# sb17v/GaussianK-SGD

Hardware: AMD Instinct MI355X
Metric: images/sec (whole node) ResNet-50 k=0.1% at 1/2/4/8 MI355X; effective grad compression ratio (higher is better)
Workload: dtype fp32; 1 GPU; model=resnet50, global_batch=512, per_gpu_batch=512, image_size=224, parallelism=dp1, compressor=gaussian, buckets=1, threshold=524288000, planner=threshold, exchange=local, momentum_correction=True, hip_graph=False, f32_matmul=bf16x6

## Files before the change

gaussiank_sgd_amd/ops/bn.py:

```python
from __future__ import annotations

import os
from typing import Optional

import torch
import torch.nn as nn
import torch.nn.functional as F

from . import load, require_native

_CL = torch.channels_last
_FIN_FUSE = os.environ.get("GKSGD_BN_FIN_FUSE", "0") == "1"


def _ops():
    return torch.ops.gksgd


def _grad_pair(grads, like):
    gs = [g for g in grads if g is not None]
    out = []
    for g in gs:
        g = g.contiguous(memory_format=_CL)
        if g.dtype != like.dtype:
            g = g.to(like.dtype)
        out.append(g)
    return (out + [None, None])[:2]


class BnLink:

    __slots__ = ("h", "mask", "twin", "dy2", "dz", "part", "dy2c", "geo")

    def __init__(self):
        self.h = self.mask = self.dy2 = self.dz = self.part = self.dy2c = self.geo = None
        self.twin = False

    def ready(self) -> bool:
        return self.h is not None and (not self.twin or self.dy2 is not None)

    def scatter_dy2c(self) -> Optional[torch.Tensor]:
        if self.dy2c is None:
            return None
        H, W, OH, OW = self.geo
        C = self.dy2c.shape[1]
        N = self.dy2c.shape[0] // (OH * OW)
        full = torch.empty((N, C, H, W), dtype=self.dy2c.dtype, device=self.dy2c.device, memory_format=_CL).zero_()
        full[:, :, ::2, ::2] = self.dy2c.view(N, OH, OW, C).permute(0, 3, 1, 2)
        return full

    def clear(self) -> None:
        self.h = self.mask = self.dy2 = self.dz = self.part = self.dy2c = self.geo = None


class ProducerLink:

    __slots__ = ("lazy", "dx")

    def __init__(self):
        self.lazy = None
        self.dx = None

    def matches(self, dy: torch.Tensor) -> bool:
        return self.lazy is not None and dy.data_ptr() == self.lazy[0].data_ptr() and dy.shape == self.lazy[0].shape

    def materialize(self) -> torch.Tensor:
        if self.dx is None:
            dz, x, coef, _, _ = self.lazy
            self.dx = torch.empty_like(x, memory_format=_CL)
            _ops().bn_lazy_apply(dz, x, self.dx, coef)
        return self.dx

    def clear(self) -> None:
        self.lazy = self.dx = None


def _lazy_buffers(x: torch.Tensor):
    C = x.shape[1]
    coef = torch.empty(C, 4, dtype=torch.float32, device=x.device)
    padz = torch.empty(C, dtype=x.dtype, device=x.device)
    padx = torch.empty(C, dtype=x.dtype, device=x.device)
    return coef, padz, padx


def _lazy_ok(x: torch.Tensor, plink) -> bool:
    import os
    return (plink is not None and x.dtype == torch.float32 and x.shape[1] % 64 == 0 and
            os.environ.get("GKSGD_BN_LAZY", "0") != "0")


class _BNActFn(torch.autograd.Function):
    @staticmethod
    def forward(ctx, x, residual, weight, bias, running_mean, running_var, momentum, eps, relu, direct=None,
                nbt=None, twin=False, pre=None, link=None, res_link=None, plink=None, fin=None, rbn=None):
        ctx.direct = direct
        ctx.set_materialize_grads(False)
        C = x.shape[1]
        M = x.numel() // C
        eb = x.element_size()
        y = torch.empty_like(x, memory_format=_CL)
        stats = torch.empty(4, C, dtype=torch.float32, device=x.device)
        ws = torch.empty(int(_ops().bn_workspace_floats(M, C, eb)), dtype=torch.float32, device=x.device)
        rscale, rshift, dlink = rbn if rbn is not None else (None, None, None)
        ctx.dlink = dlink
        if rbn is not None and (residual.dtype != x.dtype or not residual.is_contiguous(memory_format=_CL)):
            raise RuntimeError("deferred residual BN: the pending tensor must match x (dtype, channels-last)")
        if residual is not None and residual.dtype != x.dtype:
            residual = residual.to(x.dtype)
        if residual is not None and not residual.is_contiguous(memory_format=_CL):
            residual = residual.contiguous(memory_format=_CL)
        mask = None
        if relu:
            mask = torch.empty(int(_ops().bn_mask_bytes(M, C, eb)), dtype=torch.uint8, device=x.device)
        pre_t, pre_rows = pre if pre is not None else (None, 0)
        _ops().bn_act_forward(x, residual, y, mask, weight, bias, running_mean, running_var, stats[0], stats[1],
                              stats[2], stats[3], ws, float(eps), float(momentum), bool(relu), nbt, pre_t, pre_rows,
                              fin, rscale, rshift)
        ctx.fin = fin
        ctx.relu = bool(relu)
        ctx.has_res = residual is not None
        ctx.save_for_backward(x, mask, weight, stats[0], stats[1])
        ctx.link = link
        ctx.res_link = res_link
        ctx.plink = plink
        if link is not None:
            link.h, link.mask, link.twin = x, mask, bool(twin)
        return (y, y.view_as(y)) if twin else y

    @staticmethod
    def backward(ctx, *grads):
        x, mask, weight, mean, invstd = ctx.saved_tensors
        link, res_link, plink, dlink = ctx.link, ctx.res_link, ctx.plink, ctx.dlink
        ctx.link = ctx.res_link = ctx.plink = ctx.dlink = None
        gw, gb = ctx.direct if ctx.direct is not None else (None, None)
        lazy = _lazy_ok(x, plink) and ctx.needs_input_grad[0]
        if link is not None and link.part is not None:
            dz = grads[0]
            if dz is None or dz.data_ptr() != link.dz.data_ptr():
                raise RuntimeError("BNAct bwd_link: the linked output had another consumer")
            part, rows = link.part
            link.clear()
            g = torch.empty(2, x.shape[1], dtype=torch.float32, device=x.device)
            if lazy:
                coef, padz, padx = _lazy_buffers(x)
                _ops().bn_bwd_lazy_pre(x, part, rows, weight, mean, invstd, g[0], g[1], coef, padz, padx, gw, gb)
                plink.lazy = (dz, x, coef, padz, padx)
                dx = dz
            elif dlink is not None and ctx.needs_input_grad[1]:
                dx = torch.empty_like(x, memory_format=_CL)
                x2 = dlink.x
                dx2 = torch.empty_like(x2, memory_format=_CL)
                g2 = torch.empty(2, x2.shape[1], dtype=torch.float32, device=x.device)
                ws2 = torch.empty(int(_ops().bn_workspace_floats(x2.numel() // x2.shape[1], x2.shape[1],
                                                                 x2.element_size())),
                                  dtype=torch.float32, device=x.device)
                gw2, gb2 = dlink.direct if dlink.direct is not None else (None, None)
                _ops().bn_act_backward_pre_dual(dz, x, dx, weight, mean, invstd, g[0], g[1], part, rows, gw, gb, x2,
                                                dx2, dlink.weight, dlink.mean, dlink.invstd, g2[0], g2[1], ws2, gw2,
                                                gb2)
                dlink.dz, dlink.dx, dlink.g = dz, dx2, g2
            else:
                dx = torch.empty_like(x, memory_format=_CL)
                _ops().bn_act_backward_pre(dz, x, dx, weight, mean, invstd, g[0], g[1], part, rows, gw, gb, ctx.fin)
            dres = dz if ctx.has_res and ctx.needs_input_grad[1] else None
            if res_link is not None and dres is not None:
                res_link.dy2 = dres
            if ctx.direct is not None:
                return (dx, dres) + (None,) * 16
            dgamma = g[0] if weight is not None and ctx.needs_input_grad[2] else None
            dbeta = g[1] if ctx.needs_input_grad[3] else None
            return (dx, dres, dgamma, dbeta) + (None,) * 14
        d2c = link.scatter_dy2c() if link is not None else None
        if link is not None:
            link.clear()
        dy, dy2 = _grad_pair(tuple(grads) + (d2c,), x)
        if dy is None:
            return (None,) * 18
        C = x.shape[1]
        M = x.numel() // C
        g = torch.empty(2, C, dtype=torch.float32, device=x.device)
        ws = torch.empty(int(_ops().bn_workspace_floats(M, C, x.element_size())), dtype=torch.float32,
                         device=x.device)
        if lazy:
            dz = torch.empty_like(x, memory_format=_CL)
            coef, padz, padx = _lazy_buffers(x)
            _ops().bn_act_backward_lazy(dy, dy2, mask, x, dz, weight, mean, invstd, g[0], g[1], ws, ctx.relu, coef,
                                        padz, padx, gw, gb)
            plink.lazy = (dz, x, coef, padz, padx)
            dx = dz
            dres = dz if ctx.has_res and ctx.needs_input_grad[1] else None
        else:
            dx = torch.empty_like(x, memory_format=_CL)
            dres = torch.empty_like(x, memory_format=_CL) if ctx.has_res and ctx.needs_input_grad[1] else None
            _ops().bn_act_backward(dy, mask, x, dx, dres, weight, mean, invstd, g[0], g[1], ws, ctx.relu, gw, gb,
                                   dy2, ctx.fin)
        if res_link is not None and dres is not None:
            res_link.dy2 = dres
        if ctx.direct is not None:
            return (dx, dres) + (None,) * 16
        dgamma = g[0] if weight is not None and ctx.needs_input_grad[2] else None
        dbeta = g[1] if ctx.needs_input_grad[3] else None
        return (dx, dres, dgamma, dbeta) + (None,) * 14


class DeferLink:

    __slots__ = ("x", "weight", "mean", "invstd", "direct", "dz", "dx", "g")

    def __init__(self, x, weight, mean, invstd, direct):
        self.x, self.weight, self.mean, self.invstd, self.direct = x, weight, mean, invstd, direct
        self.dz = self.dx = self.g = None


class _BNDeferFn(torch.autograd.Function):

    @staticmethod
    def forward(ctx, x, weight, bias, running_mean, running_var, momentum, eps, stats, direct=None, nbt=None,
                pre=None, dlink=None):
        ctx.direct = direct
        ctx.set_materialize_grads(False)
        C = x.shape[1]
        M = x.numel() // C
        ws = torch.empty(int(_ops().bn_workspace_floats(M, C, x.element_size())), dtype=torch.float32,
                         device=x.device)
        pre_t, pre_rows = pre if pre is not None else (None, 0)
        _ops().bn_act_finalize(x, weight, bias, running_mean, running_var, stats[0], stats[1], stats[2], stats[3], ws,
                               float(eps), float(momentum), nbt, pre_t, pre_rows)
        ctx.save_for_backward(x, weight, stats[0], stats[1])
        ctx.dlink = dlink
        return x.view_as(x)

    @staticmethod
    def backward(ctx, dy):
        x, weight, mean, invstd = ctx.saved_tensors
        dl, ctx.dlink = ctx.dlink, None
        if dy is None:
            return (None,) * 12
        if dl is not None and dl.dx is not None and dl.dz is not None and dy.data_ptr() == dl.dz.data_ptr():
            dx, g = dl.dx, dl.g
            dl.dz = dl.dx = dl.g = None
            if ctx.direct is not None:
                return (dx,) + (None,) * 11
# ... 210 lines not shown
```

gaussiank_sgd_amd/ops/conv1x1.py:

```python
from __future__ import annotations

import os
from itertools import product
from typing import Dict

import torch
import torch.nn as nn
import torch.nn.functional as F

from . import autotune
from . import load
from . import streams
from . import weight_prep
from .autotune import (X6, f32_matmul, load_choices, save_choices, set_f32_matmul,
                       tuned_choices, tuning_log)

_CL = torch.channels_last
_ENABLED = os.environ.get("GKSGD_FASTCONV", "1") != "0"
_BIAS_COLSUM = os.environ.get("GKSGD_CONV_BIAS_COLSUM", "1") != "0"
_WINO = os.environ.get("GKSGD_WINO", "1") != "0"
_FORCE = os.environ.get("GKSGD_CONV_FORCE", "")
_WINO_GRIDS = (0, 1 << 20)
_zeros: Dict[torch.device, torch.Tensor] = {}

# ... 129 lines not shown
def _lz_kw(lz, rows: bool = False) -> dict:
    _, x, coef, padz, padx = lz
    return dict(lz_x=_rows(x) if rows else x, lz_coef=coef, lz_padz=padz, lz_padx=padx)


def _dgrad(dy: torch.Tensor, w: torch.Tensor, x_shape, s: int, lz=None, plink=None, wp: bool = False) -> torch.Tensor:
    N, C, H, W, K, k, p, OH, OW = _geom(x_shape, w, s)
    g = _g()
    dt = dy.dtype
    xs = torch.empty(x_shape, dtype=dt, device=dy.device, memory_format=_CL)
    kw = _lz_kw(lz, rows=(s == 1 and k == 1)) if lz is not None else {}

    def miopen():
        return torch.ops.aten.convolution_backward(dy, xs, w, None, [s, s], [p, p], [1, 1], False, [0, 0], 1,
                                                   [True, False, False])[0]
    cands = []
    split = []
    dx = None
    if s == 2:
        dx = xs
        z = _zero(dy.device)
        run = lambda c, mb: g.conv_dgrad_s2(dy, w, dx, z, c, mb, **kw)
        cands = autotune.hip_cands(run, product(autotune.nt_cfgs(dt), autotune.NT_GRIDS))
    if s == 1:
        dx = xs
        if k == 1:
            DY, DX = _rows(dy), _rows(dx)
            Wt = _lazy(lambda: weight_prep.transposed_1x1(w, wp))
            run = lambda c, mb: g.gemm_nt(DY, Wt(), DX, c, mb, **kw)
            if lz is None:
                split = autotune.splitk_cfgs(dt, N * H * W, C, K)
        else:
            wf = _lazy(lambda: weight_prep.flipped_3x3(w, wp))
            z = _zero(dy.device)
            run = lambda c, mb: g.conv_nt(dy, wf(), dx, z, 1, p, c, mb, **kw)
        cands = autotune.hip_cands(run, product(autotune.nt_cfgs(dt), autotune.NT_GRIDS))
        cands += autotune.hip_cands(run, product(split, autotune.SPLITK_GRIDS))
    if lz is not None:
        cands.append((("mat", 0, 0), lambda: _dgrad(plink.materialize(), w, x_shape, s, wp=wp)))
        ch = autotune.pick(("dgrad", N, C, H, W, K, k, s) + autotune.dkey(dt) + ("lz",), cands)
        if ch[0] == "mat":
            return _dgrad(plink.materialize(), w, x_shape, s, wp=wp)
        run(ch[1], ch[2])
        return dx
    wino = _wino_ok(dt, k, s, K, C) and _wino_shape_fits(N, H, W, C, K)
    if wino:
        cands += _wino_cands(dy, w, dx, True, wp=wp)
    cands.append((("miopen", 0, 0), miopen))
    ch = autotune.pick(_dgrad_key(N, C, H, W, K, k, s, dt), _forced(cands))
    if ch[0] == "miopen":
        return miopen().contiguous(memory_format=_CL)
    if ch[0] in ("wino", "wx6"):
        dict(cands)[ch]()
        return dx
    run(ch[1], ch[2])
    return dx


_WGRAD_AFTER = os.environ.get("GKSGD_WGRAD_AFTER_DGRAD", "0") == "1"
_SIDE_QROUNDS = int(os.environ.get("GKSGD_WGRAD_SIDE_QROUNDS", "0"))
_FORK_BIAS = os.environ.get("GKSGD_WGRAD_STREAM_BIAS", "0") == "1"
_FORKABLE = tuple(k for k in os.environ.get("GKSGD_WGRAD_STREAM_KINDS", "hip,w3,wino").split(",")
                  if k and (k != "wino" or os.environ.get("GKSGD_WGRAD_STREAM_WINO", "1") == "1"))


def _lazy(make):
    box = []

    def get():
        if not box:
            box.append(make())
        return box[0]
    return get


def _dgrad_key(N, C, H, W, K, k, s, dt) -> tuple:
    wino = _wino_ok(dt, k, s, K, C) and _wino_shape_fits(N, H, W, C, K)
    return ("dgrad", N, C, H, W, K, k, s) + autotune.dkey(dt) + (_wino_tag(K, C) if wino else ())


def _dgrad_bn(dy: torch.Tensor, w: torch.Tensor, x_shape, s: int, link, lz=None, plink=None,
              wp: bool = False) -> torch.Tensor:
    N, C, H, W, K, k, p, OH, OW = _geom(x_shape, w, s)
    kw = _lz_kw(lz, rows=(k == 1)) if lz is not None else {}
    g = _g()
    M = N * H * W
    dt = dy.dtype
    dz = torch.empty(x_shape, dtype=dt, device=dy.device, memory_format=_CL)
    st = torch.empty(2, min(1280, (M + 63) // 64), C, dtype=torch.float32, device=dy.device)
    h, mask, dy2 = link.h, link.mask, link.dy2
    if k == 1:
        DY, DZ = _rows(dy), _rows(dz)
        Wt = _lazy(lambda: weight_prep.transposed_1x1(w, wp))
        H2 = _rows(h)
        D2 = _rows(dy2) if dy2 is not None else None
        run = lambda c, mb: g.gemm_nt(DY, Wt(), DZ, c, mb, st, None, H2, D2, mask, **kw)
        split = autotune.splitk_cfgs(dt, M, C, K) if lz is None else []
    else:
        split = []
        wf = _lazy(lambda: weight_prep.flipped_3x3(w, wp))
        z = _zero(dy.device)
        run = lambda c, mb: g.conv_nt(dy, wf(), dz, z, 1, p, c, mb, st, None, h, dy2, mask, **kw)
    bn_cfgs = [c for c in autotune.nt_cfgs(dt) if c % 10 <= 4 or c >= 1000]
    cands = autotune.hip_cands(run, product(bn_cfgs, autotune.NT_GRIDS))
    cands += autotune.hip_cands(run, product(split, autotune.SPLITK_GRIDS))
    key = ("dgrad_bn", N, C, H, W, K, k, s, dy2 is not None) + autotune.dkey(dt)
    if lz is not None:
        cands.append((("mat", 0, 0), lambda: _dgrad_bn(plink.materialize(), w, x_shape, s, link, wp=wp)))
        ch = autotune.pick(key + ("lz",), cands)
        if ch[0] == "mat":
            return _dgrad_bn(plink.materialize(), w, x_shape, s, link, wp=wp)
    else:
        if _wino_ok(dt, k, s, K, C) and _wino_shape_fits(N, H, W, C, K):
            cands += _wino_cands(dy, w, dz, True, st, (h, dy2, mask), wp=wp)
            key = key + _wino_tag(K, C)
        ch = autotune.pick(key, _forced(cands))
    if ch[0] in ("wino", "wx6"):
        rows = dict(cands)[ch]()
    else:
        rows = run(ch[1], ch[2])
    link.part = (st, int(rows))
    link.dz = dz
    return dz


def _link_on(ds: bool = False) -> bool:
    return os.environ.get("GKSGD_BN_LINK", "1") != "0" and \
        not (ds and os.environ.get("GKSGD_BN_LINK_DS", "1") == "0")


def _ds_compact_ok(ds_link, x: torch.Tensor, w: torch.Tensor, s: int, dt: torch.dtype) -> bool:
    return (ds_link is not None and s == 2 and w.shape[2] == 1 and dt == torch.float32 and _link_on(ds=True) and
            f32_matmul() == "bf16x6" and ds_link.h is not None and ds_link.h.dtype == dt and
            ds_link.h.shape == x.shape and ds_link.dy2 is None and ds_link.dy2c is None and
            x.numel() // x.shape[1] < (1 << 31))


def _dgrad_ds(dy: torch.Tensor, w: torch.Tensor, x_shape, wp: bool = False) -> torch.Tensor:
    N, C, H, W, K, k, p, OH, OW = _geom(x_shape, w, 2)
    g = _g()
    dt = dy.dtype
    dxc = torch.empty(N * OH * OW, C, dtype=dt, device=dy.device)
    DY = _rows(dy)
    Wt = _lazy(lambda: weight_prep.transposed_1x1(w, wp))
    run = lambda c, mb: g.gemm_nt(DY, Wt(), dxc, c, mb)
    cands = autotune.hip_cands(run, product(autotune.nt_cfgs(dt), autotune.NT_GRIDS))
    cands += autotune.hip_cands(run, product(autotune.splitk_cfgs(dt, N * OH * OW, C, K), autotune.SPLITK_GRIDS))
    ch = autotune.pick(("dgrad_ds", N, C, H, W, K) + autotune.dkey(dt), cands)
    run(ch[1], ch[2])
    return dxc


def _ds_fusable(link, x: torch.Tensor, w: torch.Tensor, s: int, dt: torch.dtype, dgrad_key: tuple, lz) -> bool:
    if not (s == 1 and w.shape[2] == 1 and dt == torch.float32 and lz is None and _link_on(ds=True) and
            f32_matmul() == "bf16x6" and link.h is not None and link.h.dtype == dt and link.h.shape == x.shape):
        return False
    ch = autotune.choice(dgrad_key)
    return ch is None or ch[0] == "hip"


def _dgrad_bn_ds(dy: torch.Tensor, w: torch.Tensor, x_shape, link, wp: bool = False) -> torch.Tensor:
    N, C, H, W, K, k, p, OH, OW = _geom(x_shape, w, 1)
    g = _g()
    M = N * H * W
    dt = dy.dtype
    dz = torch.empty(x_shape, dtype=dt, device=dy.device, memory_format=_CL)
    st = torch.empty(2, min(1280, (M + 63) // 64), C, dtype=torch.float32, device=dy.device)
    DY, DZ, H2 = _rows(dy), _rows(dz), _rows(link.h)
    D2, geo, mask = link.dy2c, list(link.geo), link.mask
    Wt = _lazy(lambda: weight_prep.transposed_1x1(w, wp))
    run = lambda c, mb: g.gemm_nt(DY, Wt(), DZ, c, mb, st, None, H2, D2, mask, bn_dy2_geo=geo)
    cands = autotune.hip_cands(run, product(autotune.nt_x62_cfgs(), autotune.NT_GRIDS))
    ch = autotune.pick(("dgrad_bn_ds", N, C, H, W, K) + autotune.dkey(dt), cands)
    rows = run(ch[1], ch[2])
    link.part = (st, int(rows))
    link.dz = dz
    link.dy2c = None
    return dz


def _bn_fusable(link, s: int, dgrad_key: tuple) -> bool:
    if link is None or s != 1 or not _link_on() or not link.ready():
        return False
    if link.h.dtype != dgrad_key_dtype(dgrad_key):
        return False
    ch = autotune.choice(dgrad_key)
    return ch is None or ch[0] in ("hip", "wino", "wx6")


def dgrad_key_dtype(key: tuple) -> torch.dtype:
    return torch.float32 if "f32" in key[8:] else torch.bfloat16


def _wgrad_key(x: torch.Tensor, w: torch.Tensor, s: int, lz=None) -> tuple:
    N, C, H, W, K, k, p, OH, OW = _geom(x.shape, w, s)
    wino = lz is None and _wino_ok(x.dtype, k, s, C, K) and C % 64 == 0 and _wino_shape_fits(N, H, W, C, K)
    return ("wgrad", N, C, H, W, K, k, s) + autotune.dkey(x.dtype) + (("lz",) if lz is not None else ()) + \
        (("wino",) if wino else ())


def _wgrad_into(dy: torch.Tensor, x: torch.Tensor, w: torch.Tensor, s: int, out_f32: torch.Tensor, lz=None,
                plink=None, side: bool = False) -> None:
    N, C, H, W, K, k, p, OH, OW = _geom(x.shape, w, s)
    g = _g()
# ... 247 lines not shown
```

gaussiank_sgd_amd/ops/csrc/bindings.cpp:

```cpp
#include <ATen/ATen.h>
#include <c10/core/DeviceGuard.h>
#include <c10/hip/HIPStream.h>
#include <torch/custom_class.h>
#include <torch/library.h>

#include <cstring>
#include <vector>

#include "comm/rccl_engine.h"
#include "kernels/gemm_cfg.h"
#include "kernels/gk_kernels.h"

namespace {

hipStream_t cur_stream(const at::Tensor& t) {
  return c10::hip::getCurrentHIPStream(t.device().index()).stream();
}

void check_dev(const at::Tensor& t, const char* name) {
  TORCH_CHECK(t.is_cuda(), name, " must be a GPU tensor");
  TORCH_CHECK(t.is_contiguous(), name, " must be contiguous");
}

void check_f32(const at::Tensor& t, const char* name) {
// ... 511 lines not shown
  return (int64_t)gk::bn_mask_bytes(M, (int)C, (int)elem_bytes);
}

void* fin_state(const OptTensor& fin, int C) {
  if (!has(fin)) return nullptr;
  TORCH_CHECK(fin->is_cuda() && fin->is_contiguous() && fin->nbytes() >= gk::bn_fin_state_bytes(C) &&
                  reinterpret_cast<uintptr_t>(fin->data_ptr()) % 16 == 0,
              "fin: a contiguous, 16-byte aligned GPU tensor of bn_fin_state_bytes(C) bytes");
  return fin->data_ptr();
}

int64_t bn_fin_state_bytes(int64_t C) { return (int64_t)gk::bn_fin_state_bytes((int)C); }

void bn_act_forward(at::Tensor x, OptTensor res, at::Tensor y, OptTensor mask, OptTensor w, OptTensor b,
                    OptTensor run_mean, OptTensor run_var, at::Tensor save_mean, at::Tensor save_invstd,
                    at::Tensor scale, at::Tensor shift, at::Tensor ws, double eps, double momentum, bool relu,
                    OptTensor nbt, OptTensor pre, int64_t pre_rows, OptTensor fin, OptTensor rscale,
                    OptTensor rshift) {
  const gk::BnShape sh = bn_shape(x);
  check_same(x, {&y}, "y");
  gk::BnResidual r{opt_same(x, res, "residual"), nullptr, nullptr};
  TORCH_CHECK(has(rscale) == has(rshift), "rscale and rshift go together");
  if (has(rscale)) {
    TORCH_CHECK(r.res != nullptr, "rscale / rshift need a residual");
    r.rscale = opt_channel_buf(rscale, sh.C, "rscale");
    r.rshift = opt_channel_buf(rshift, sh.C, "rshift");
  }
  const gk::BnFwdStats st =
      fwd_stats(w, b, run_mean, run_var, save_mean, save_invstd, scale, shift, eps, momentum, nbt, sh.C);
  float* wp = check_ws(ws, sh);
  uint8_t* mp = relu_mask(mask, relu, sh);
  const gk::BnPartials p = partials(pre, pre_rows, sh.C, "pre");
  void* fs = fin_state(fin, sh.C);
  c10::DeviceGuard guard(x.device());
  gk::bn_act_forward(sh, x.data_ptr(), r, y.data_ptr(), mp, st, p, wp, relu ? 1 : 0, fs, cur_stream(x));
}

void bn_act_finalize(at::Tensor x, OptTensor w, OptTensor b, OptTensor run_mean, OptTensor run_var,
                     at::Tensor save_mean, at::Tensor save_invstd, at::Tensor scale, at::Tensor shift, at::Tensor ws,
                     double eps, double momentum, OptTensor nbt, OptTensor pre, int64_t pre_rows) {
  const gk::BnShape sh = bn_shape(x);
  const gk::BnFwdStats st =
      fwd_stats(w, b, run_mean, run_var, save_mean, save_invstd, scale, shift, eps, momentum, nbt, sh.C);
  float* wp = check_ws(ws, sh);
  const gk::BnPartials p = partials(pre, pre_rows, sh.C, "pre");
  c10::DeviceGuard guard(x.device());
  gk::bn_act_finalize(sh, x.data_ptr(), st, p, wp, cur_stream(x));
}

void bn_act_backward(at::Tensor dy, OptTensor mask, at::Tensor x, at::Tensor dx, OptTensor dres, OptTensor w,
                     at::Tensor mean, at::Tensor invstd, at::Tensor dgamma, at::Tensor dbeta, at::Tensor ws, bool relu,
                     OptTensor gw_acc, OptTensor gb_acc, OptTensor dy2, OptTensor fin) {
  const gk::BnShape sh = bn_shape(x);
  check_same(x, {&dy}, "dy");
  check_same(x, {&dx}, "dx");
  void* rp = opt_same(x, dres, "dres");
  const void* d2 = opt_dy2(dy2, dy);
  const gk::BnBwdStats bs = bwd_stats(w, mean, invstd, dgamma, dbeta, gw_acc, gb_acc, sh.C);
  float* wp = check_ws(ws, sh);
  const uint8_t* mp = relu_mask(mask, relu, sh);
  void* fs = fin_state(fin, sh.C);
  c10::DeviceGuard guard(x.device());
  gk::bn_act_backward(sh, dy.data_ptr(), d2, mp, x.data_ptr(), dx.data_ptr(), rp, bs, wp, relu ? 1 : 0, fs,
                      cur_stream(x));
}

void bn_act_backward_pre(at::Tensor dz, at::Tensor x, at::Tensor dx, OptTensor w, at::Tensor mean, at::Tensor invstd,
                         at::Tensor dgamma, at::Tensor dbeta, at::Tensor part, int64_t rows, OptTensor gw_acc,
                         OptTensor gb_acc, OptTensor fin) {
  const gk::BnShape sh = bn_shape(x);
  check_same(x, {&dz}, "dz");
  check_same(x, {&dx}, "dx");
  const gk::BnBwdStats bs = bwd_stats(w, mean, invstd, dgamma, dbeta, gw_acc, gb_acc, sh.C);
  const gk::BnPartials p = partials(part, rows, sh.C, "part");
  void* fs = fin_state(fin, sh.C);
  c10::DeviceGuard guard(x.device());
  gk::bn_act_backward_pre(sh, dz.data_ptr(), x.data_ptr(), dx.data_ptr(), bs, p, fs, cur_stream(x));
}

void bn_act_backward_pre_dual(at::Tensor dz, at::Tensor x, at::Tensor dx, OptTensor w, at::Tensor mean,
                              at::Tensor invstd, at::Tensor dgamma, at::Tensor dbeta, at::Tensor part, int64_t rows,
                              OptTensor gw_acc, OptTensor gb_acc, at::Tensor x2, at::Tensor dx2, OptTensor w2,
                              at::Tensor mean2, at::Tensor invstd2, at::Tensor dgamma2, at::Tensor dbeta2,
                              at::Tensor ws2, OptTensor gw2_acc, OptTensor gb2_acc) {
  const gk::BnShape sh = bn_shape(x);
  check_same(x, {&dz, &dx, &x2, &dx2}, "dz / dx / x2 / dx2");
  const gk::BnBwdStats bs = bwd_stats(w, mean, invstd, dgamma, dbeta, gw_acc, gb_acc, sh.C);
  const gk::BnBwdStats bs2 = bwd_stats(w2, mean2, invstd2, dgamma2, dbeta2, gw2_acc, gb2_acc, sh.C);
  const gk::BnPartials p = partials(part, rows, sh.C, "part");
  float* wp2 = check_ws(ws2, sh);
  c10::DeviceGuard guard(x.device());
  gk::bn_act_backward_pre_dual(sh, dz.data_ptr(), x.data_ptr(), dx.data_ptr(), bs, p, x2.data_ptr(), dx2.data_ptr(),
                               bs2, wp2, cur_stream(x));
}

gk::BnLazyOut lazy_out(const at::Tensor& x, int C, const at::Tensor& coef, const at::Tensor& padz,
                       const at::Tensor& padx) {
  TORCH_CHECK(coef.is_cuda() && coef.scalar_type() == at::kFloat && coef.is_contiguous() && coef.numel() >= 4 * C,
              "coef must be a contiguous fp32 [C, 4] GPU tensor");
  for (const at::Tensor* t : {&padz, &padx})
    TORCH_CHECK(t->is_cuda() && t->scalar_type() == x.scalar_type() && t->is_contiguous() && t->numel() >= C,
                "padz / padx must be contiguous [C] GPU tensors of x's dtype");
  return {coef.data_ptr<float>(), padz.data_ptr(), padx.data_ptr()};
}

void bn_bwd_lazy_pre(at::Tensor x, at::Tensor part, int64_t rows, OptTensor w, at::Tensor mean, at::Tensor invstd,
                     at::Tensor dgamma, at::Tensor dbeta, at::Tensor coef, at::Tensor padz, at::Tensor padx,
                     OptTensor gw_acc, OptTensor gb_acc) {
  const gk::BnShape sh = bn_shape(x);
  const gk::BnPartials p = partials(part, rows, sh.C, "part");
  const gk::BnBwdStats bs = bwd_stats(w, mean, invstd, dgamma, dbeta, gw_acc, gb_acc, sh.C);
  const gk::BnLazyOut lz = lazy_out(x, sh.C, coef, padz, padx);
  c10::DeviceGuard guard(x.device());
  gk::bn_bwd_finalize_lazy(sh, p, 1, bs, lz, cur_stream(x));
}

void bn_act_backward_lazy(at::Tensor dy, OptTensor dy2, OptTensor mask, at::Tensor x, at::Tensor dz, OptTensor w,
                          at::Tensor mean, at::Tensor invstd, at::Tensor dgamma, at::Tensor dbeta, at::Tensor ws,
                          bool relu, at::Tensor coef, at::Tensor padz, at::Tensor padx, OptTensor gw_acc,
                          OptTensor gb_acc) {
  const gk::BnShape sh = bn_shape(x);
  check_same(x, {&dy}, "dy");
  check_same(x, {&dz}, "dz");
  const void* d2 = opt_dy2(dy2, dy);
  const gk::BnBwdStats bs = bwd_stats(w, mean, invstd, dgamma, dbeta, gw_acc, gb_acc, sh.C);
  float* wp = check_ws(ws, sh);
  const uint8_t* mp = relu_mask(mask, relu, sh);
  const gk::BnLazyOut lz = lazy_out(x, sh.C, coef, padz, padx);
  c10::DeviceGuard guard(x.device());
  gk::bn_act_backward_lazy(sh, dy.data_ptr(), d2, mp, x.data_ptr(), dz.data_ptr(), bs, wp, relu ? 1 : 0, lz,
                           cur_stream(x));
}

void bn_stats_partials(at::Tensor x, at::Tensor ws) {
  const gk::BnShape sh = bn_shape(x);
  float* wp = check_ws(ws, sh);
  c10::DeviceGuard guard(x.device());
  gk::bn_stats_partials(sh, x.data_ptr(), wp, cur_stream(x));
}

void bn_lazy_apply(at::Tensor dz, at::Tensor x, at::Tensor dx, at::Tensor coef) {
  const gk::BnShape sh = bn_shape(x);
  check_same(x, {&dz}, "dz");
  check_same(x, {&dx}, "dx");
  TORCH_CHECK(coef.is_cuda() && coef.scalar_type() == at::kFloat && coef.is_contiguous() && coef.numel() >= 4 * sh.C,
              "coef must be a contiguous fp32 [C, 4] GPU tensor");
  c10::DeviceGuard guard(x.device());
  gk::bn_lazy_apply(sh, dz.data_ptr(), x.data_ptr(), dx.data_ptr(), coef.data_ptr<float>(), cur_stream(x));
}

gk::PoolGeo pool_geo(const at::Tensor& x, const at::Tensor& y, const char* y_name, int64_t k, int64_t st,
                     int64_t pad) {
  check_cl(y, y_name);
  TORCH_CHECK(x.dim() == 4 && y.dim() == 4 && x.size(0) == y.size(0) && x.size(1) == y.size(1) &&
                  y.scalar_type() == x.scalar_type(),
              y_name, " must be 4-D with x's batch, channels and dtype");
  gk::PoolGeo pg;
  pg.H = (int)x.size(2);
  pg.W = (int)x.size(3);
  pg.OH = (int)y.size(2);
  pg.OW = (int)y.size(3);
  pg.k = (int)k;
  pg.s = (int)st;
  pg.p = (int)pad;
  TORCH_CHECK(k >= 1 && k <= 15 && st >= 1 && pad >= 0 && 2 * pad <= k, "unsupported pool window");
  TORCH_CHECK(pg.OH == (pg.H + 2 * pg.p - pg.k) / pg.s + 1 && pg.OW == (pg.W + 2 * pg.p - pg.k) / pg.s + 1,
              "pool output shape mismatch (ceil_mode unsupported)");
  TORCH_CHECK(x.numel() / x.size(1) < (int64_t(1) << 32), "N*H*W must be < 2^32");
  return pg;
}

uint8_t* pool_amax(const at::Tensor& amax, const at::Tensor& y) {
  TORCH_CHECK(amax.is_cuda() && amax.scalar_type() == at::kByte && amax.numel() >= y.numel(),
              "amax: a uint8 GPU tensor of the pooled tensor's element count");
  return amax.data_ptr<uint8_t>();
}
// ... 111 lines not shown
  void init_async(at::Tensor uid, int64_t rank, int64_t world, int64_t device) {
    TORCH_CHECK(!uid.is_cuda() && uid.scalar_type() == at::kByte, "uid must be a CPU uint8 tensor");
    at::Tensor c = uid.contiguous();
    std::vector<uint8_t> v(c.data_ptr<uint8_t>(), c.data_ptr<uint8_t>() + c.numel());
    comm.init_async(v, (int)rank, (int)world, (int)device);
  }
  int64_t init_poll() { return comm.init_poll(); }
  void init_wait(double timeout_s) { comm.init_wait(timeout_s); }
  void abort() { comm.abort(); }
  void set_op_timeout(double s) { comm.set_op_timeout(s); }

  void allgather(at::Tensor send, at::Tensor recv) {
    check_dev(send, "send");
    check_dev(recv, "recv");
    TORCH_CHECK(recv.nbytes() == send.nbytes() * (size_t)comm.world(), "recv must be world x send bytes");
    c10::DeviceGuard guard(send.device());
    comm.allgather_bytes(send.data_ptr(), recv.data_ptr(), send.nbytes(), cur_stream(send));
  }

  void allreduce(at::Tensor t, int64_t op) {
    check_dev(t, "t");
    c10::DeviceGuard guard(t.device());
    ncclRedOp_t o = op == 0 ? ncclSum : (op == 1 ? ncclAvg : (op == 2 ? ncclMax : ncclMin));
    comm.allreduce(t.data_ptr(), (size_t)t.numel(), to_nccl(t.scalar_type()), o, cur_stream(t));
  }

  void broadcast(at::Tensor t, int64_t root) {
    check_dev(t, "t");
    c10::DeviceGuard guard(t.device());
    comm.broadcast(t.data_ptr(), (size_t)t.numel(), to_nccl(t.scalar_type()), (int)root, cur_stream(t));
  }

  void allgather_many(std::vector<at::Tensor> sends, std::vector<at::Tensor> recvs) {
    TORCH_CHECK(sends.size() == recvs.size() && !sends.empty(), "allgather_many: matching non-empty lists");
    std::vector<const void*> sp;
    std::vector<void*> rp;
    std::vector<size_t> nb;
    for (size_t i = 0; i < sends.size(); ++i) {
      check_dev(sends[i], "send");
      check_dev(recvs[i], "recv");
      TORCH_CHECK(sends[i].device() == sends[0].device() && recvs[i].device() == sends[0].device(),
                  "allgather_many: one device");
      TORCH_CHECK(recvs[i].nbytes() == sends[i].nbytes() * (size_t)comm.world(), "recv must be world x send bytes");
      sp.push_back(sends[i].data_ptr());
      rp.push_back(recvs[i].data_ptr());
      nb.push_back(sends[i].nbytes());
    }
    c10::DeviceGuard guard(sends[0].device());
    comm.allgather_many(sp, rp, nb, cur_stream(sends[0]));
  }

  void inject_failure(std::string why) { comm.inject_failure(why); }
  void destroy() { comm.destroy(); }
  int64_t rank() const { return comm.rank(); }
  int64_t world() const { return comm.world(); }

  void set_tracking(bool on) { comm.set_tracking(on); }
  void start_watchdog(double timeout_s, double poll_ms) { comm.start_watchdog(timeout_s, poll_ms); }
  void stop_watchdog() { comm.stop_watchdog(); }
  int64_t poll() { return comm.poll(); }
  bool failed() const { return comm.failed(); }
  std::string error() const { return comm.error(); }
  void check() const { comm.check(); }
  int64_t in_flight() const { return comm.in_flight(); }
  void reset_stats() { comm.reset_stats(); }
  std::vector<double> stats(int64_t op) const {
    gk::OpStats st = comm.stats((int)op);
    return {(double)st.calls, (double)st.bytes, st.ms_total, st.ms_max};
  }
};

bool gemm_supported(int64_t N, int64_t K) { return gk::gemm_supported(N, K); }

bool is_gemm_dtype(const at::Tensor& t) { return t.scalar_type() == at::kBFloat16 || t.scalar_type() == at::kFloat; }

void check_rows(const at::Tensor& t, const char* name, const at::Tensor& like) {
  TORCH_CHECK(t.is_cuda() && is_gemm_dtype(t) && t.scalar_type() == like.scalar_type() && t.dim() == 2, name,
              " must be a 2-D bf16 or fp32 GPU tensor (all operands one dtype)");
  TORCH_CHECK(t.stride(1) == 1 && (t.stride(0) * t.element_size()) % 16 == 0, name,
              " rows must be contiguous, 16-byte aligned");
  TORCH_CHECK(reinterpret_cast<uintptr_t>(t.data_ptr()) % 16 == 0, name, " must be 16-byte aligned");
}

float* stats_ptr(const c10::optional<at::Tensor>& st, int64_t N, int* rows) {
  if (!st.has_value()) {
    *rows = 0;
    return nullptr;
  }
  const at::Tensor& t = *st;
  TORCH_CHECK(t.is_cuda() && t.scalar_type() == at::kFloat && t.is_contiguous() && t.dim() == 3 && t.size(0) == 2 &&
                  t.size(2) == N && t.size(1) > 0,
              "stats must be a contiguous fp32 [2, rows, N] GPU tensor");
  *rows = (int)t.size(1);
  return t.data_ptr<float>();
}

void check_stem_x(const at::Tensor& x) {
  TORCH_CHECK(x.is_cuda() && x.dim() == 4 && x.size(1) == 3 &&
                  (x.scalar_type() == at::kFloat || x.scalar_type() == at::kBFloat16) &&
                  x.is_contiguous(at::MemoryFormat::ChannelsLast),
              "stem: x must be a channels-last fp32 / bf16 [N, 3, H, W] GPU tensor");
  TORCH_CHECK(gk::stem_supported((int)x.size(2), (int)x.size(3)), "stem: unsupported image size");
  TORCH_CHECK(x.size(0) * x.size(2) * x.size(3) < (int64_t(1) << 31), "stem: batch too large");
}

void stem_pack(at::Tensor w, at::Tensor wp) {
  TORCH_CHECK(w.is_cuda() && w.scalar_type() == at::kFloat && w.dim() == 4 && w.size(0) == 64 && w.size(1) == 3 &&
                  w.size(2) == 7 && w.size(3) == 7,
              "stem_pack: w must be fp32 [64, 3, 7, 7]");
  TORCH_CHECK(wp.is_cuda() && wp.scalar_type() == at::kBFloat16 && wp.is_contiguous() && wp.numel() == 64 * 224,
              "stem_pack: wp must be contiguous bf16 [64, 224]");
  c10::DeviceGuard guard(w.device());
  gk::stem_pack_weight(w.data_ptr<float>(), w.stride(0), w.stride(1), w.stride(2), w.stride(3),
                       static_cast<uint16_t*>(wp.data_ptr()), cur_stream(w));
}

int64_t stem_fwd(at::Tensor x, at::Tensor wp, at::Tensor y, c10::optional<at::Tensor> stats) {
  check_stem_x(x);
  const int64_t N = x.size(0), H = x.size(2), W = x.size(3);
  const int64_t OH = (H - 1) / 2 + 1, OW = (W - 1) / 2 + 1;
  TORCH_CHECK(wp.is_cuda() && wp.scalar_type() == at::kBFloat16 && wp.is_contiguous() && wp.numel() == 64 * 224,
              "stem_fwd: wp must be the packed bf16 [64, 224] weights");
  TORCH_CHECK(y.is_cuda() && y.scalar_type() == at::kBFloat16 && y.dim() == 4 && y.size(0) == N && y.size(1) == 64 &&
                  y.size(2) == OH && y.size(3) == OW && y.is_contiguous(at::MemoryFormat::ChannelsLast),
              "stem_fwd: y must be channels-last bf16 [N, 64, OH, OW]");
  int rows = 0;
  float* sp = stats_ptr(stats, 64, &rows);
  c10::DeviceGuard guard(x.device());
  return gk::stem_forward(x.data_ptr(), x.scalar_type() == at::kFloat, (int)N, (int)H, (int)W,
                          static_cast<const uint16_t*>(wp.data_ptr()), static_cast<uint16_t*>(y.data_ptr()), sp, rows,
                          cur_stream(x));
}

int64_t stem_wgrad_ws(int64_t N, int64_t H, int64_t W) {
  return (int64_t)gk::stem_wgrad_blocks((int)N, (int)H, (int)W) * 64 * 224;
}

void stem_wgrad(at::Tensor x, at::Tensor dy, at::Tensor out, at::Tensor part) {
  check_stem_x(x);
  const int64_t N = x.size(0), H = x.size(2), W = x.size(3);
  const int64_t OH = (H - 1) / 2 + 1, OW = (W - 1) / 2 + 1;
  TORCH_CHECK(dy.is_cuda() && dy.scalar_type() == at::kBFloat16 && dy.dim() == 4 && dy.size(0) == N &&
                  dy.size(1) == 64 && dy.size(2) == OH && dy.size(3) == OW &&
                  dy.is_contiguous(at::MemoryFormat::ChannelsLast),
              "stem_wgrad: dy must be channels-last bf16 [N, 64, OH, OW]");
  TORCH_CHECK(out.is_cuda() && out.scalar_type() == at::kFloat && out.dim() == 4 && out.size(0) == 64 &&
                  out.size(1) == 3 && out.size(2) == 7 && out.size(3) == 7,
              "stem_wgrad: out must be fp32 [64, 3, 7, 7]");
  TORCH_CHECK(part.is_cuda() && part.scalar_type() == at::kFloat && part.is_contiguous() &&
                  part.numel() >= stem_wgrad_ws(N, H, W),
              "stem_wgrad: part must hold stem_wgrad_ws(N, H, W) floats");
  c10::DeviceGuard guard(x.device());
  gk::stem_wgrad(x.data_ptr(), x.scalar_type() == at::kFloat, (int)N, (int)H, (int)W,
                 static_cast<const uint16_t*>(dy.data_ptr()), part.data_ptr<float>(), out.data_ptr<float>(),
                 out.stride(0), out.stride(1), out.stride(2), out.stride(3), cur_stream(x));
}

int64_t stem_f32_fwd(at::Tensor x, at::Tensor w, at::Tensor y, c10::optional<at::Tensor> stats) {
  TORCH_CHECK(x.is_cuda() && x.scalar_type() == at::kFloat && x.dim() == 4 && x.size(1) == 3 &&
                  x.is_contiguous(at::MemoryFormat::ChannelsLast) && gk::stem_f32_supported((int)x.size(2), (int)x.size(3)) &&
                  reinterpret_cast<uintptr_t>(x.data_ptr()) % 16 == 0,
              "stem_f32_fwd: x must be a channels-last fp32 [N, 3, 224, 224] GPU tensor (16-byte aligned)");
  TORCH_CHECK(w.is_cuda() && w.scalar_type() == at::kFloat && w.dim() == 4 && w.size(0) == 64 && w.size(1) == 3 &&
                  w.size(2) == 7 && w.size(3) == 7, "stem_f32_fwd: w must be fp32 [64, 3, 7, 7]");
  const int64_t N = x.size(0);
  TORCH_CHECK(y.is_cuda() && y.scalar_type() == at::kFloat && y.dim() == 4 && y.size(0) == N && y.size(1) == 64 &&
                  y.size(2) == 112 && y.size(3) == 112 && y.is_contiguous(at::MemoryFormat::ChannelsLast),
              "stem_f32_fwd: y must be a channels-last fp32 [N, 64, 112, 112] GPU tensor");
  int rows = 0;
  float* sp = stats_ptr(stats, 64, &rows);
  c10::DeviceGuard guard(x.device());
  return gk::stem_f32_forward(x.data_ptr<float>(), (int)N, (int)x.size(2), (int)x.size(3), w.data_ptr<float>(),
                              w.stride(0), w.stride(1), w.stride(2), w.stride(3), y.data_ptr<float>(), sp, rows,
                              cur_stream(x));
}

int64_t stem_f32x6_wplanes() { return gk::stem_f32x6_wplanes(); }

int64_t stem_f32x6_fwd(at::Tensor x, at::Tensor w, at::Tensor y, c10::optional<at::Tensor> stats, at::Tensor wp3) {
  TORCH_CHECK(x.is_cuda() && x.scalar_type() == at::kFloat && x.dim() == 4 && x.size(1) == 3 &&
                  x.is_contiguous(at::MemoryFormat::ChannelsLast) && gk::stem_f32_supported((int)x.size(2), (int)x.size(3)) &&
                  reinterpret_cast<uintptr_t>(x.data_ptr()) % 16 == 0,
              "stem_f32x6_fwd: x must be a channels-last fp32 [N, 3, 224, 224] GPU tensor (16-byte aligned)");
  TORCH_CHECK(w.is_cuda() && w.scalar_type() == at::kFloat && w.dim() == 4 && w.size(0) == 64 && w.size(1) == 3 &&
                  w.size(2) == 7 && w.size(3) == 7, "stem_f32x6_fwd: w must be fp32 [64, 3, 7, 7]");
  const int64_t N = x.size(0);
  TORCH_CHECK(y.is_cuda() && y.scalar_type() == at::kFloat && y.dim() == 4 && y.size(0) == N && y.size(1) == 64 &&
                  y.size(2) == 112 && y.size(3) == 112 && y.is_contiguous(at::MemoryFormat::ChannelsLast),
              "stem_f32x6_fwd: y must be a channels-last fp32 [N, 64, 112, 112] GPU tensor");
  TORCH_CHECK(wp3.is_cuda() && wp3.scalar_type() == at::kBFloat16 && wp3.is_contiguous() &&
                  wp3.numel() >= gk::stem_f32x6_wplanes() && reinterpret_cast<uintptr_t>(wp3.data_ptr()) % 16 == 0,
              "stem_f32x6_fwd: wp3 must be a contiguous bf16 GPU tensor of stem_f32x6_wplanes() elements");
  int rows = 0;
  float* sp = stats_ptr(stats, 64, &rows);
  c10::DeviceGuard guard(x.device());
  return gk::stem_f32x6_forward(x.data_ptr<float>(), (int)N, (int)x.size(2), (int)x.size(3), w.data_ptr<float>(),
                                w.stride(0), w.stride(1), w.stride(2), w.stride(3),
                                static_cast<uint16_t*>(wp3.data_ptr()), y.data_ptr<float>(), sp, rows, cur_stream(x));
}

int64_t stem_f32_wgrad_ws(int64_t N) { return (int64_t)gk::stem_f32_wgrad_blocks((int)N) * 64 * 148; }

void stem_f32_wgrad(at::Tensor x, at::Tensor dy, at::Tensor out, at::Tensor part, bool x6) {
  TORCH_CHECK(x.is_cuda() && x.scalar_type() == at::kFloat && x.dim() == 4 && x.size(1) == 3 &&
                  x.is_contiguous(at::MemoryFormat::ChannelsLast) && gk::stem_f32_supported((int)x.size(2), (int)x.size(3)) &&
                  reinterpret_cast<uintptr_t>(x.data_ptr()) % 16 == 0,
              "stem_f32_wgrad: x must be a channels-last fp32 [N, 3, 224, 224] GPU tensor (16-byte aligned)");
  const int64_t N = x.size(0);
  TORCH_CHECK(dy.is_cuda() && dy.scalar_type() == at::kFloat && dy.dim() == 4 && dy.size(0) == N &&
                  dy.size(1) == 64 && dy.size(2) == 112 && dy.size(3) == 112 &&
                  dy.is_contiguous(at::MemoryFormat::ChannelsLast),
              "stem_f32_wgrad: dy must be a channels-last fp32 [N, 64, 112, 112] GPU tensor");
  TORCH_CHECK(out.is_cuda() && out.scalar_type() == at::kFloat && out.dim() == 4 && out.size(0) == 64 &&
                  out.size(1) == 3 && out.size(2) == 7 && out.size(3) == 7, "stem_f32_wgrad: out must be fp32 [64, 3, 7, 7]");
  TORCH_CHECK(part.is_cuda() && part.scalar_type() == at::kFloat && part.is_contiguous() &&
                  part.numel() >= stem_f32_wgrad_ws(N), "stem_f32_wgrad: part must hold stem_f32_wgrad_ws(N) floats");
  c10::DeviceGuard guard(x.device());
  gk::stem_f32_wgrad(x.data_ptr<float>(), dy.data_ptr<float>(), (int)N, (int)x.size(2), (int)x.size(3),
                     part.data_ptr<float>(), out.data_ptr<float>(), out.stride(0), out.stride(1), out.stride(2),
                     out.stride(3), x6, cur_stream(x));
}

const uint32_t* seed_word(const c10::optional<at::Tensor>& t) {
  if (!t.has_value() || !t->defined()) return nullptr;
  TORCH_CHECK(t->is_cuda() && t->scalar_type() == at::kInt && t->numel() >= 1, "seed_dev must be a GPU int32[>=1]");
  return reinterpret_cast<const uint32_t*>(t->data_ptr<int32_t>());
}

const float* bias_ptr(const c10::optional<at::Tensor>& b, int64_t N) {
  if (!b.has_value() || !b->defined()) return nullptr;
  TORCH_CHECK(b->is_cuda() && b->scalar_type() == at::kFloat && b->is_contiguous() && b->numel() == N,
              "bias must be a contiguous fp32 [N] GPU tensor");
  return b->data_ptr<float>();
}

bool bn_bwd_args(const c10::optional<at::Tensor>& h, const c10::optional<at::Tensor>& dy2,
                 const c10::optional<at::Tensor>& mask, int64_t M, int64_t N,
                 int64_t ldc, bool has_stats, at::ScalarType dt, gk::BnBwdArgs* out,
                 c10::OptionalArrayRef<int64_t> dy2_geo = c10::nullopt) {
  const bool compact = dy2_geo.has_value();
  if (!h.has_value() || !h->defined()) {
    TORCH_CHECK(!compact, "bn_dy2_geo needs the BN-backward epilogue operands");
    return false;
  }
  TORCH_CHECK(has_stats, "BN-backward epilogue needs the stats partials buffer");
  auto rows_ok = [&](const at::Tensor& t, const char* what) {
    TORCH_CHECK(t.is_cuda() && t.scalar_type() == dt && t.numel() == M * N &&
                    (t.dim() == 2 ? t.stride(0) == ldc && t.stride(1) == 1
                                  : t.is_contiguous(at::MemoryFormat::ChannelsLast) && ldc == N),
                what, " must have C's dtype, shape and row stride");
  };
  rows_ok(*h, "bn h");
  out->h = h->data_ptr();
  out->dy2 = nullptr;
  out->H = out->W = out->OH = out->OW = 0;
  if (compact) {
    TORCH_CHECK(dy2_geo->size() == 4 && dy2.has_value() && dy2->defined(), "bn_dy2_geo is [H, W, OH, OW] of a given bn_dy2");
    const int64_t H = (*dy2_geo)[0], W = (*dy2_geo)[1], OH = (*dy2_geo)[2], OW = (*dy2_geo)[3];
    TORCH_CHECK(H > 0 && W > 0 && OH == (H + 1) / 2 && OW == (W + 1) / 2 && M % (H * W) == 0 && M < (int64_t(1) << 31),
                "bn_dy2_geo: OH x OW must be the stride-2 grid of the H x W pixels of C's rows (M < 2^31)");
    TORCH_CHECK(dt == at::kFloat && dy2->is_cuda() && dy2->scalar_type() == dt && dy2->dim() == 2 &&
                    dy2->size(0) == M / (H * W) * OH * OW && dy2->size(1) == N && dy2->stride(0) == ldc &&
                    dy2->stride(1) == 1,
                "compact bn dy2 must be fp32 [M / (H W) * OH * OW, N] with C's row stride");
    out->dy2 = dy2->data_ptr();
    out->H = (int)H, out->W = (int)W, out->OH = (int)OH, out->OW = (int)OW;
  } else if (dy2.has_value() && dy2->defined()) {
    rows_ok(*dy2, "bn dy2");
    out->dy2 = dy2->data_ptr();
  }
  out->mask = nullptr;
  if (mask.has_value() && mask->defined()) {
    const int64_t V = dt == at::kFloat ? 4 : 8;
    TORCH_CHECK(mask->is_cuda() && mask->scalar_type() == at::kByte && mask->numel() >= M * (N / V),
                "bn mask must hold M * N / V bytes");
    out->mask = mask->data_ptr<uint8_t>();
  }
  return true;
}

bool lazy_args(const c10::optional<at::Tensor>& x, const c10::optional<at::Tensor>& coef,
               const c10::optional<at::Tensor>& padz, const c10::optional<at::Tensor>& padx, const at::Tensor& dz,
               int64_t C, gk::LazyArgs* out) {
  if (!x.has_value() || !x->defined()) return false;
  TORCH_CHECK(dz.scalar_type() == at::kFloat, "lazy BN operand: fp32 kernels only");
  TORCH_CHECK(x->is_cuda() && x->scalar_type() == dz.scalar_type() && x->sizes() == dz.sizes() &&
                  x->strides() == dz.strides(),
              "lz_x must match the dz operand's dtype, shape and strides");
  TORCH_CHECK(coef.has_value() && coef->defined() && coef->is_cuda() && coef->scalar_type() == at::kFloat &&
                  coef->is_contiguous() && coef->numel() >= 4 * C,
              "lz_coef must be a contiguous fp32 [C, 4] GPU tensor");
  for (const c10::optional<at::Tensor>* t : {&padz, &padx})
    TORCH_CHECK(t->has_value() && (*t)->defined() && (*t)->is_cuda() && (*t)->scalar_type() == dz.scalar_type() &&
                    (*t)->is_contiguous() && (*t)->numel() >= C,
                "lz_padz / lz_padx must be contiguous [C] GPU tensors of dz's dtype");
  TORCH_CHECK(C > 0 && C % 64 == 0, "lazy BN operand: channels must be a multiple of 64");
  out->x = x->data_ptr();
  out->coef = coef->data_ptr<float>();
  out->padz = padz->data_ptr();
  out->padx = padx->data_ptr();
  out->C = (int)C;
  return true;
}

struct NtWordAux {
  at::Tensor ws, b3;
  NtWordAux(const char* op, const gk::cfg::NtWord& w, bool gather, bool f32, bool has_lz, const at::Tensor& B,
            int64_t ldb, int64_t M, int64_t N, int64_t K, int64_t C, hipStream_t stream) {
    if (w.planes > 1) {
      TORCH_CHECK(f32 && !has_lz && w.planes <= 16 && gk::cfg::splitk_divides(w.planes, gather, (int)K, (int)C), op,
                  " split-K: fp32, no lazy operand, S <= 16 ", gather ? "dividing the K slices" : "and K % (64 S) == 0");
      ws = at::empty({w.planes, M, N}, B.options().dtype(at::kFloat));
    }
    if (w.family == 3) {
      TORCH_CHECK(B.scalar_type() == at::kFloat && (gather || K % 32 == 0), op, ": cfg family 3 takes fp32 operands");
      b3 = at::empty({N, 3 * K}, B.options().dtype(at::kBFloat16));
      gk::split3_rows(B.data_ptr<float>(), ldb, b3.data_ptr(), N, (int)K, stream);
    }
  }
  float* ws_ptr() const { return ws.defined() ? ws.data_ptr<float>() : nullptr; }
  const void* b3_ptr() const { return b3.defined() ? b3.data_ptr() : nullptr; }
  static int64_t checked(const char* op, int r) {
    TORCH_CHECK(r != gk::cfg::kRowGemmsOnly, op,
                ": the register-staged bf16x6 kernels (cfg digit 200000/300000) take plain row GEMMs only");
    TORCH_CHECK(r != gk::cfg::kCompactDy2, op,
                ": a compact bn_dy2 takes one register-staged bf16x6 row GEMM (cfg digit 200000/300000, no split-K)");
    TORCH_CHECK(r >= 0, op, ": the lazy operand's coefficient table does not fit this tile configuration");
    return r;
  }
};

int64_t gemm_nt(at::Tensor A, at::Tensor B, at::Tensor C, int64_t cfg, int64_t max_blocks,
                c10::optional<at::Tensor> stats, c10::optional<at::Tensor> bias, c10::optional<at::Tensor> bn_h,
                c10::optional<at::Tensor> bn_dy2, c10::optional<at::Tensor> bn_mask, c10::optional<at::Tensor> lz_x, c10::optional<at::Tensor> lz_coef,
                c10::optional<at::Tensor> lz_padz, c10::optional<at::Tensor> lz_padx,
                c10::OptionalArrayRef<int64_t> bn_dy2_geo) {
  check_rows(A, "A", A);
  check_rows(B, "B", A);
  check_rows(C, "C", A);
  const int64_t M = A.size(0), K = A.size(1), N = B.size(0);
  TORCH_CHECK(B.size(1) == K && C.size(0) == M && C.size(1) == N, "gemm_nt: shape mismatch");
  TORCH_CHECK(gk::gemm_supported(N, K), "gemm_nt: N and K must be multiples of 64");
  TORCH_CHECK(M > 0, "gemm_nt: empty M");
  int rows = 0;
  float* sp = stats_ptr(stats, N, &rows);
  gk::BnBwdArgs bn{};
  const bool has_bn = bn_bwd_args(bn_h, bn_dy2, bn_mask, M, N, C.stride(0), sp != nullptr, C.scalar_type(), &bn,
                                  bn_dy2_geo);
  TORCH_CHECK(!has_bn || !bias.has_value() || !bias->defined(), "gemm_nt: bias and BN epilogue are exclusive");
  gk::LazyArgs lz{};
  const bool has_lz = lazy_args(lz_x, lz_coef, lz_padz, lz_padx, A, K, &lz);
  c10::DeviceGuard guard(A.device());
  const bool f32 = A.scalar_type() == at::kFloat;
  const NtWordAux aux("gemm_nt", gk::cfg::NtWord::decode((int)cfg), false, f32, has_lz, B, B.stride(0), M, N, K, K,
                      cur_stream(A));
  const int r = gk::gemm_nt(A.data_ptr(), A.stride(0), B.data_ptr(), B.stride(0), C.data_ptr(), C.stride(0), M, (int)N,
                            (int)K, f32, (int)cfg, (int)max_blocks, sp, rows, bias_ptr(bias, N),
                            has_bn ? &bn : nullptr, has_lz ? &lz : nullptr, cur_stream(A), aux.ws_ptr(), aux.b3_ptr());
  return NtWordAux::checked("gemm_nt", r);
}

void gemm_tn_acc(at::Tensor G, at::Tensor X, at::Tensor W, int64_t cfg, int64_t splits, c10::optional<at::Tensor> lz_x, c10::optional<at::Tensor> lz_coef,
                c10::optional<at::Tensor> lz_padz, c10::optional<at::Tensor> lz_padx) {
  check_rows(G, "G", G);
  check_rows(X, "X", G);
  TORCH_CHECK(W.is_cuda() && W.scalar_type() == at::kFloat && W.dim() == 2 && W.stride(1) == 1,
              "W must be a 2-D fp32 GPU tensor with contiguous rows");
  const int64_t M = G.size(0), N = G.size(1), K = X.size(1);
  TORCH_CHECK(X.size(0) == M && W.size(0) == N && W.size(1) == K, "gemm_tn_acc: shape mismatch");
  TORCH_CHECK(gk::gemm_supported(N, K), "gemm_tn_acc: N and K must be multiples of 64");
  if (M == 0) return;
  gk::LazyArgs lz{};
  const bool has_lz = lazy_args(lz_x, lz_coef, lz_padz, lz_padx, G, N, &lz);
  c10::DeviceGuard guard(G.device());
  const int rc = gk::gemm_tn_acc(G.data_ptr(), G.stride(0), X.data_ptr(), X.stride(0), W.data_ptr<float>(), W.stride(0), M, (int)N,
                  (int)K, G.scalar_type() == at::kFloat, (int)cfg, (int)splits, has_lz ? &lz : nullptr, cur_stream(G));
  TORCH_CHECK(rc != gk::cfg::kRowGemmsOnly, "gemm_tn_acc: the register-staged bf16x6 kernels (cfg digit 200000) take plain row GEMMs only");
}

void check_zero(const at::Tensor& zero) {
  TORCH_CHECK(zero.is_cuda() && zero.is_contiguous() && zero.numel() * zero.element_size() >= 128,
              "zero must hold >= 128 zero bytes");
}

void check_conv(const at::Tensor& x, const at::Tensor& w, const at::Tensor& zero) {
  TORCH_CHECK(x.is_cuda() && is_gemm_dtype(x) && x.dim() == 4 && x.is_contiguous(at::MemoryFormat::ChannelsLast),
              "conv: x must be a channels-last bf16 or fp32 GPU tensor");
  TORCH_CHECK(w.is_cuda() && w.scalar_type() == x.scalar_type() && w.dim() == 4 &&
                  w.is_contiguous(at::MemoryFormat::ChannelsLast) && w.size(1) == x.size(1),
              "conv: w must be a channels-last [Cout, C, KH, KW] GPU tensor of x's dtype");
  TORCH_CHECK(x.size(1) % 64 == 0 && w.size(0) % 64 == 0, "conv: C and Cout must be multiples of 64");
  check_zero(zero);
}

int64_t conv_nt(at::Tensor x, at::Tensor w, at::Tensor y, at::Tensor zero, int64_t stride, int64_t pad, int64_t cfg,
                int64_t max_blocks, c10::optional<at::Tensor> stats, c10::optional<at::Tensor> bias,
                c10::optional<at::Tensor> bn_h, c10::optional<at::Tensor> bn_dy2, c10::optional<at::Tensor> bn_mask,
                c10::optional<at::Tensor> lz_x, c10::optional<at::Tensor> lz_coef,
                c10::optional<at::Tensor> lz_padz, c10::optional<at::Tensor> lz_padx) {
  check_conv(x, w, zero);
  const int64_t N = x.size(0), C = x.size(1), H = x.size(2), W = x.size(3);
  const int64_t Co = w.size(0), KH = w.size(2), KW = w.size(3);
  const int64_t OH = (H + 2 * pad - KH) / stride + 1, OW = (W + 2 * pad - KW) / stride + 1;
  TORCH_CHECK(KH <= 4 && KW <= 4, "conv_nt: kernels up to 4x4 (gemm.hip kMaxTaps)");
  TORCH_CHECK(y.is_cuda() && y.scalar_type() == x.scalar_type() && y.dim() == 4 &&
                  y.is_contiguous(at::MemoryFormat::ChannelsLast) && y.size(0) == N && y.size(1) == Co &&
                  y.size(2) == OH && y.size(3) == OW,
              "conv_nt: y must be channels-last [N, Cout, OH, OW] of x's dtype");
  const int64_t M = N * OH * OW;
  TORCH_CHECK(M > 0 && M < (int64_t(1) << 32), "conv_nt: M out of range");
  int rows = 0;
  float* sp = stats_ptr(stats, Co, &rows);
  gk::BnBwdArgs bn{};
  const bool has_bn = bn_bwd_args(bn_h, bn_dy2, bn_mask, M, Co, Co, sp != nullptr, y.scalar_type(), &bn);
  TORCH_CHECK(!has_bn || !bias.has_value() || !bias->defined(), "conv_nt: bias and BN epilogue are exclusive");
  gk::LazyArgs lz{};
  const bool has_lz = lazy_args(lz_x, lz_coef, lz_padz, lz_padx, x, C, &lz);
  c10::DeviceGuard guard(x.device());
  const bool f32 = x.scalar_type() == at::kFloat;
  const int64_t K = KH * KW * C;
  const NtWordAux aux("conv_nt", gk::cfg::NtWord::decode((int)cfg), true, f32, has_lz, w, K, M, Co, K, C, cur_stream(x));
  const int r = gk::conv_nt(x.data_ptr(), zero.data_ptr(), (int)H, (int)W, (int)C, (int)OH, (int)OW, (int)stride,
                            (int)pad, (int)KH, (int)KW, w.data_ptr(), y.data_ptr(), M, (int)Co, f32, (int)cfg,
                            (int)max_blocks, sp, rows, bias_ptr(bias, Co), has_bn ? &bn : nullptr,
                            has_lz ? &lz : nullptr, cur_stream(x), aux.ws_ptr(), aux.b3_ptr());
  return NtWordAux::checked("conv_nt", r);
}

int64_t weight_prep_blocks(int64_t kind, int64_t R, int64_t S) { return gk::weight_prep_blocks((int)kind, (int)R, (int)S); }

void weight_prep(at::Tensor table, int64_t ndesc, int64_t total_blocks) {
// ... 668 lines not shown
    gk::lstm_cell_bwd(static_cast<const uint16_t*>(po), static_cast<const uint16_t*>(pr), pp, (int)S, pc,
                      gates.data_ptr<float>(), c.data_ptr<float>(), c_prev.data_ptr<float>(),
                      static_cast<uint16_t*>(dG.data_ptr()), static_cast<uint16_t*>(gp), dc_prev.data_ptr<float>(),
                      (int)B, (int)H, (int)Hp, cur_stream(gates));
}

}


TORCH_LIBRARY(gksgd, m) {
  m.def("ctrl_bytes() -> int", &ctrl_bytes);
  m.def("workspace_bytes() -> int", &workspace_bytes);
  m.def(
      "compress(Tensor(a!) g, Tensor(b!) r, Tensor(c!) ctrl, Tensor(d!) ws, Tensor(e!) record, int mode, bool ec, "
      "bool zero_g, int loops, float z, float fixed_thr, float sample_p, int k, int k_cap, int seed, "
      "int n_stats, Tensor(f!)? stats_out=None, Tensor? valid=None, Tensor(g!)? u=None, Tensor? w=None, "
      "Tensor? chunks=None, int chunk_begin=0, int chunk_count=0, int chunk_base=0, float[] mc_mu=[], "
      "float[] mc_wd=[], Tensor? seed_dev=None, int handoff=-1) -> ()");
  m.def("apply_records_sgd(Tensor(a!) w, Tensor(b!)? w_bf16, Tensor records, int P, int k_cap, float scale, float lr, "
        "Tensor? lr_mult=None) -> ()");
  m.def("arena_digest(Tensor x, Tensor(a!) out, Tensor(b!) ws) -> ()");
  m.def("tensor_stats(Tensor x, Tensor(a!) ctrl, Tensor(b!) ws) -> ()");
  m.def("quality_workspace_bytes() -> int", &quality_workspace_bytes);
  m.def("selection_quality(Tensor r, Tensor record, int k, int k_cap, Tensor(a!) out, Tensor(b!) ws) -> ()");
  m.def("scatter_add_records(Tensor(a!) dst, Tensor records, int P, int k_cap, float scale, bool deterministic) -> ()");
  m.def("fill_zero(Tensor(a!) dst) -> ()");
  m.def("sign_bucket_workspace_bytes() -> int", &sign_bucket_workspace_bytes);
  m.def("sign_bucket_compress(Tensor(a!) x, Tensor(b!) mask, Tensor(c!) means, Tensor(d!) ws) -> ()");
  m.def("sign_bucket_decompress(Tensor(a!) x, Tensor mask, Tensor means) -> ()");
  m.def(
      "fused_sgd(Tensor(a!) w, Tensor(b!)? m, Tensor(c!) g, Tensor chunks, float[] lr, float[] momentum, "
      "float[] dampening, float[] weight_decay, int[] nesterov, int[] first_step, bool zero_grad, "
      "Tensor? grad_scale=None, Tensor(d!)? w_bf16=None, Tensor? lr_mult=None) -> ()");
  m.def(
      "fused_adam(Tensor(a!) w, Tensor(b!) m, Tensor(c!) v, Tensor(d!) g, Tensor chunks, Tensor(e!) step, float[] lr, "
      "float[] beta1, float[] beta2, float[] eps, float[] weight_decay, int[] decoupled, bool zero_grad, "
      "Tensor? grad_scale=None, Tensor(f!)? w_bf16=None, Tensor? lr_mult=None) -> ()");
  m.def(
      "fused_lamb(Tensor(a!) w, Tensor(b!) m, Tensor(c!) v, Tensor(d!) g, Tensor chunks, Tensor(e!) step, "
      "Tensor seg_range, Tensor(f!) part, Tensor(g!) trust, float[] lr, float[] beta1, float[] beta2, float[] eps, "
      "float[] weight_decay, int[] adapt, float[] trust_clip, bool zero_grad, Tensor? grad_scale=None, "
      "Tensor(h!)? w_bf16=None, Tensor? lr_mult=None, int passes=7) -> ()");
  m.def("segmented_sumsq(Tensor w, Tensor g, Tensor chunks, Tensor(a!) out) -> ()");
  m.def(
      "fused_lars(Tensor(a!) w, Tensor(b!) m, Tensor g, Tensor chunks, Tensor seg_sumsq, float[] lr, "
      "float[] momentum, float[] weight_decay, float[] eeta, float[] epsilon) -> ()");
  m.def("clip_grad_norm(Tensor(a!) g, float max_norm, Tensor(b!) ws, Tensor(c!) coef, Tensor(d!) norm) -> ()");

  m.def("bn_workspace_floats(int M, int C, int elem_bytes) -> int", &bn_workspace_floats);
  m.def("bn_supported(int C, int elem_bytes) -> bool", &bn_supported);
  m.def("bn_set_blocks(int blocks) -> ()", [](int64_t b) { gk::bn_set_blocks((int)b); });
  m.def("bn_mask_bytes(int M, int C, int elem_bytes) -> int", &bn_mask_bytes);
  m.def(
      "bn_act_forward(Tensor x, Tensor? res, Tensor(a!) y, Tensor(i!)? mask, Tensor? w, Tensor? b, Tensor(b!)? run_mean, "
      "Tensor(c!)? run_var, Tensor(d!) save_mean, Tensor(e!) save_invstd, Tensor(f!) scale, Tensor(g!) shift, "
      "Tensor(h!) ws, float eps, float momentum, bool relu, Tensor(j!)? nbt=None, Tensor? pre=None, "
      "int pre_rows=0, Tensor(k!)? fin=None, Tensor? rscale=None, Tensor? rshift=None) -> ()");
  m.def(
      "bn_act_finalize(Tensor x, Tensor? w, Tensor? b, Tensor(a!)? run_mean, Tensor(b!)? run_var, "
      "Tensor(c!) save_mean, Tensor(d!) save_invstd, Tensor(e!) scale, Tensor(f!) shift, Tensor(g!) ws, float eps, "
      "float momentum, Tensor(h!)? nbt=None, Tensor? pre=None, int pre_rows=0) -> ()");
  m.def(
      "bn_relu_pool_forward(Tensor x, Tensor(a!) y, Tensor(b!) amax, Tensor? w, Tensor? b, Tensor(c!)? run_mean, "
      "Tensor(d!)? run_var, Tensor(e!) save_mean, Tensor(f!) save_invstd, Tensor(g!) scale, Tensor(h!) shift, "
      "Tensor(i!) ws, float eps, float momentum, int k, int s, int p, Tensor(j!)? nbt=None, Tensor? pre=None, "
      "int pre_rows=0) -> ()");
  m.def(
      "bn_relu_pool_backward(Tensor dy, Tensor amax, Tensor x, Tensor(a!) dx, Tensor? w, Tensor mean, "
      "Tensor invstd, Tensor(b!) dgamma, Tensor(c!) dbeta, Tensor(d!) ws, int k, int s, int p, "
      "Tensor(e!)? gw_acc=None, Tensor(f!)? gb_acc=None, Tensor? dy2=None) -> ()");
  m.def(
      "bn_act_backward(Tensor dy, Tensor? mask, Tensor x, Tensor(a!) dx, Tensor(b!)? dres, Tensor? w, Tensor mean, "
      "Tensor invstd, Tensor(c!) dgamma, Tensor(d!) dbeta, Tensor(e!) ws, bool relu, Tensor(f!)? gw_acc=None, "
      "Tensor(g!)? gb_acc=None, Tensor? dy2=None, Tensor(h!)? fin=None) -> ()");
  m.def("accum_grad(Tensor(a!) dst, Tensor src) -> ()");
  m.def(
      "momentum_correct(Tensor(a!) u, Tensor(b!) g, Tensor w, Tensor chunks, int begin, int count, "
      "float[] momentum, float[] weight_decay) -> ()");
  m.def("mask_records(Tensor(a!) u, Tensor record, int k_cap) -> ()");
  m.def("cast_bf16(Tensor(a!) dst, Tensor src) -> ()");
  m.def("gemm_supported(int N, int K) -> bool", &gemm_supported);
  m.def("gemm_nt(Tensor A, Tensor B, Tensor(a!) C, int cfg=0, int max_blocks=0, Tensor(b!)? stats=None, "
        "Tensor? bias=None, Tensor? bn_h=None, Tensor? bn_dy2=None, Tensor? bn_mask=None, Tensor? lz_x=None, Tensor? lz_coef=None, Tensor? lz_padz=None, Tensor? lz_padx=None, "
        "int[]? bn_dy2_geo=None) -> int");
  m.def("gemm_tn_acc(Tensor G, Tensor X, Tensor(a!) W, int cfg=0, int splits=0, Tensor? lz_x=None, Tensor? lz_coef=None, Tensor? lz_padz=None, Tensor? lz_padx=None) -> ()");
  m.def("conv_nt(Tensor x, Tensor w, Tensor(a!) y, Tensor zero, int stride, int pad, int cfg=0, int max_blocks=0, "
        "Tensor(b!)? stats=None, Tensor? bias=None, Tensor? bn_h=None, Tensor? bn_dy2=None, Tensor? bn_mask=None, "
        "Tensor? lz_x=None, Tensor? lz_coef=None, Tensor? lz_padz=None, Tensor? lz_padx=None) -> int");
  m.def("stem_supported(int H, int W) -> bool", [](int64_t H, int64_t W) { return gk::stem_supported((int)H, (int)W); });
  m.def("stem_wgrad_ws(int N, int H, int W) -> int", &stem_wgrad_ws);
  m.def("stem_pack(Tensor w, Tensor(a!) wp) -> ()");
  m.def("stem_fwd(Tensor x, Tensor wp, Tensor(a!) y, Tensor(b!)? stats=None) -> int");
  m.def("stem_wgrad(Tensor x, Tensor dy, Tensor(a!) out, Tensor(b!) part) -> ()");
  m.def("stem_f32_supported(int H, int W) -> bool", [](int64_t H, int64_t W) { return gk::stem_f32_supported((int)H, (int)W); });
  m.def("stem_f32_fwd(Tensor x, Tensor w, Tensor(a!) y, Tensor(b!)? stats=None) -> int");
  m.def("stem_f32x6_wplanes() -> int", &stem_f32x6_wplanes);
  m.def("stem_f32x6_fwd(Tensor x, Tensor w, Tensor(a!) y, Tensor(b!)? stats, Tensor(c!) wp3) -> int");
  m.def("stem_f32_wgrad_ws(int N) -> int", &stem_f32_wgrad_ws);
  m.def("stem_f32_wgrad(Tensor x, Tensor dy, Tensor(a!) out, Tensor(b!) part, bool x6=False) -> ()");
  m.def("wgrad3_supported(int H, int W, int C, int K) -> bool", [](int64_t H, int64_t W, int64_t C, int64_t K) {
    return gk::wgrad3_supported((int)H, (int)W, (int)C, (int)K);
  });
  m.def("wgrad3_ws(int N, int H, int W, int C, int K) -> int", &wgrad3_ws);
  m.def("conv3_wgrad(Tensor dy, Tensor x, Tensor(a!) out, Tensor(b!) part, Tensor zero) -> ()");
  m.def("wino_weights(Tensor w, Tensor(a!) u, bool flip) -> ()");
  m.def("weight_prep(Tensor table, int ndesc, int total_blocks) -> ()");
  m.def("weight_prep_blocks(int kind, int R, int S) -> int", &weight_prep_blocks);
  m.def("wino_wgrad_ws(int N, int H, int W, int C, int K, int splits=0) -> int", &wino_wgrad_ws);
  m.def("wino_wgrad(Tensor x, Tensor dy, Tensor(a!) out, Tensor(b!) part, int splits=0) -> ()");
  m.def("wino_conv(Tensor x, Tensor u, Tensor(a!) y, int max_blocks=0, Tensor(b!)? stats=None, Tensor? bn_h=None, "
        "Tensor? bn_dy2=None, Tensor? bn_mask=None, int splits=1) -> int");
  m.def("wino_x6_weights(Tensor w, Tensor(a!) u3, bool flip) -> ()");
  m.def("wino_x6_conv(Tensor x, Tensor u3, Tensor(a!) y, int max_blocks=0, Tensor(b!)? stats=None, "
        "Tensor? bn_h=None, Tensor? bn_dy2=None, Tensor? bn_mask=None) -> int");
  m.def("conv_dgrad_s2(Tensor dy, Tensor w, Tensor(a!) dx, Tensor zero, int cfg=0, int max_blocks=0, "
        "Tensor? lz_x=None, Tensor? lz_coef=None, Tensor? lz_padz=None, Tensor? lz_padx=None) -> ()");
  m.def("bn_bwd_lazy_pre(Tensor x, Tensor part, int rows, Tensor? w, Tensor mean, Tensor invstd, "
        "Tensor(a!) dgamma, Tensor(b!) dbeta, Tensor(c!) coef, Tensor(d!) padz, Tensor(e!) padx, "
        "Tensor(f!)? gw_acc=None, Tensor(g!)? gb_acc=None) -> ()");
  m.def("bn_act_backward_lazy(Tensor dy, Tensor? dy2, Tensor? mask, Tensor x, Tensor(a!) dz, Tensor? w, "
        "Tensor mean, Tensor invstd, Tensor(b!) dgamma, Tensor(c!) dbeta, Tensor(d!) ws, bool relu, "
        "Tensor(e!) coef, Tensor(f!) padz, Tensor(g!) padx, Tensor(h!)? gw_acc=None, Tensor(i!)? gb_acc=None) -> ()");
  m.def("bn_lazy_apply(Tensor dz, Tensor x, Tensor(a!) dx, Tensor coef) -> ()");
  m.def("bn_stats_partials(Tensor x, Tensor(a!) ws) -> ()");
  m.def(
      "bn_act_backward_pre_dual(Tensor dz, Tensor x, Tensor(a!) dx, Tensor? w, Tensor mean, Tensor invstd, "
      "Tensor(b!) dgamma, Tensor(c!) dbeta, Tensor part, int rows, Tensor(d!)? gw_acc, Tensor(e!)? gb_acc, Tensor x2, "
      "Tensor(f!) dx2, Tensor? w2, Tensor mean2, Tensor invstd2, Tensor(g!) dgamma2, Tensor(h!) dbeta2, "
      "Tensor(i!) ws2, Tensor(j!)? gw2_acc, Tensor(k!)? gb2_acc) -> ()");
  m.def("bn_act_backward_pre(Tensor dz, Tensor x, Tensor(a!) dx, Tensor? w, Tensor mean, Tensor invstd, "
        "Tensor(b!) dgamma, Tensor(c!) dbeta, Tensor part, int rows, Tensor(d!)? gw_acc=None, "
        "Tensor(e!)? gb_acc=None, Tensor(f!)? fin=None) -> ()");
  m.def("bn_fin_state_bytes(int C) -> int", &bn_fin_state_bytes);
  m.def("attn_supported(int T, int D) -> bool",
        [](int64_t T, int64_t D) { return gk::attn_supported((int)T, (int)D); });
  m.def("attn_fwd(Tensor qkv, Tensor(a!) out, Tensor(b!) lse, int heads, float p, int seed, Tensor? seed_dev=None, "
        "Tensor? key_bits=None, Tensor(c!)? out_lo=None, bool causal=False) -> ()");
  m.def("attn_pack_key_mask(Tensor mask, Tensor(a!) bits) -> ()");
  m.def("attn_bwd(Tensor qkv, Tensor out, Tensor dout, Tensor lse, Tensor(a!) delta, Tensor(b!) dqkv, int heads, "
        "float p, int seed, Tensor? seed_dev=None, Tensor? key_bits=None, Tensor? out_lo=None, "
        "bool causal=False) -> ()");
  m.def("attn_dropout_mask(Tensor(a!) mask, int B, int heads, int T, float p, int seed, Tensor? seed_dev=None) -> ()");
  m.def("attn_f32_fwd(Tensor qkv, Tensor(a!) out, Tensor(b!) lse, int heads, float p, int seed, Tensor? seed_dev=None, "
        "Tensor? key_bits=None, bool causal=False) -> ()");
  m.def("attn_f32_bwd(Tensor qkv, Tensor out, Tensor dout, Tensor lse, Tensor(a!) delta, Tensor(b!) dqkv, int heads, "
        "float p, int seed, Tensor? seed_dev=None, Tensor? key_bits=None, bool causal=False) -> ()");
  m.def("attn_f32_supported(int T, int D) -> bool",
        [](int64_t T, int64_t D) { return gk::attn_f32_supported((int)T, (int)D); });
  m.def("add_ln_supported(int H) -> bool", &add_ln_supported);
  m.def("add_ln_ws_floats(int R, int H) -> int", &add_ln_ws_floats);
  m.def("xent_supported(int V) -> bool", &xent_supported);
  m.def("xent_forward(Tensor logits, Tensor labels, Tensor(a!) lse, Tensor(b!) loss, int ignore) -> ()");
  m.def("xent_backward(Tensor logits, Tensor labels, Tensor lse, Tensor scale, Tensor(a!) grad, int ignore) -> ()");
  m.def("emb_supported(int H, int NT) -> bool", &emb_supported);
  m.def("emb_part_floats(int H) -> int", &emb_part_floats);
  m.def("emb_forward(Tensor ids, Tensor? tt, Tensor Ww, Tensor Wp, Tensor Wt, Tensor(a!) out) -> ()");
  m.def("emb_word_ws_ints(int V, int M) -> int", &emb_word_ws_ints);
  m.def("emb_word_part_floats(int M, int H) -> int", &emb_word_part_floats);
  m.def("emb_backward(Tensor ids, Tensor? tt, Tensor dx, Tensor(a!)? dWw, Tensor(b!)? dWp, Tensor(c!)? dWt, "
        "Tensor(d!) part, Tensor sid, Tensor order, Tensor(e!) wws, Tensor(f!) wpart) -> ()");
  m.def("add_ln_forward(Tensor a, Tensor x, Tensor? gamma, Tensor? beta, Tensor(a!) y, Tensor(b!) h, "
        "Tensor(c!) mean, Tensor(d!) rstd, float eps, float p, int seed, Tensor? seed_dev=None) -> ()");
  m.def("add_ln_backward(Tensor dy, Tensor h, Tensor mean, Tensor rstd, Tensor? gamma, Tensor(a!) dx, "
        "Tensor(b!)? da, Tensor(c!)? dgamma, Tensor(d!)? dbeta, bool accumulate, Tensor(e!) ws, float p, int seed, "
        "Tensor? seed_dev=None) -> ()");
  m.def("conv_tn_acc(Tensor dy, Tensor x, Tensor(a!) wout, Tensor zero, int stride, int pad, int cfg=0, int splits=0, "
        "Tensor? lz_x=None, Tensor? lz_coef=None, Tensor? lz_padz=None, Tensor? lz_padx=None) -> ()");
  m.def("colsum_acc(Tensor dy, Tensor(a!) db) -> ()");
  m.def("gelu_bwd_colsum(Tensor dy, Tensor pre, Tensor(a!) dpre, Tensor(b!)? db=None) -> ()");
  m.def("lstm_rec_gemm(Tensor A, Tensor B, Tensor(a!) P, int S) -> ()");
  m.def("lstm_rec_gemm_x6(Tensor A, Tensor B3, Tensor(a!) P, int S) -> ()");
  m.def("lstm_cell_fwd(Tensor xg, Tensor? hg, Tensor? P, int S, Tensor c_prev, Tensor(a!) c, Tensor(b!) h, Tensor(c!)? h_pad, "
        "Tensor(d!) gates) -> ()");
  m.def("lstm_cell_bwd(Tensor? dout, Tensor? dh_rec, Tensor? P, int S, Tensor? dc_next, Tensor gates, Tensor c, Tensor c_prev, "
        "Tensor(a!) dG, Tensor(b!)? dG_pad, Tensor(c!) dc_prev) -> ()");

  m.class_<RcclEngine>("RcclEngine")
      .def(torch::init<>())
      .def_static("unique_id", &RcclEngine::unique_id)
      .def("init", &RcclEngine::init)
      .def("init_async", &RcclEngine::init_async)
      .def("init_poll", &RcclEngine::init_poll)
      .def("init_wait", &RcclEngine::init_wait)
      .def("abort", &RcclEngine::abort)
      .def("set_op_timeout", &RcclEngine::set_op_timeout)
      .def("allgather", &RcclEngine::allgather)
      .def("allreduce", &RcclEngine::allreduce)
      .def("broadcast", &RcclEngine::broadcast)
      .def("allgather_many", &RcclEngine::allgather_many)
      .def("set_tracking", &RcclEngine::set_tracking)
      .def("start_watchdog", &RcclEngine::start_watchdog)
      .def("stop_watchdog", &RcclEngine::stop_watchdog)
      .def("poll", &RcclEngine::poll)
      .def("failed", &RcclEngine::failed)
      .def("error", &RcclEngine::error)
      .def("check", &RcclEngine::check)
      .def("in_flight", &RcclEngine::in_flight)
      .def("reset_stats", &RcclEngine::reset_stats)
      .def("stats", &RcclEngine::stats)
      .def("inject_failure", &RcclEngine::inject_failure)
      .def("destroy", &RcclEngine::destroy)
      .def("rank", &RcclEngine::rank)
      .def("world", &RcclEngine::world);
}

TORCH_LIBRARY_IMPL(gksgd, CUDA, m) {
  m.impl("compress", &compress);
  m.impl("tensor_stats", &tensor_stats);
  m.impl("selection_quality", &selection_quality);
  m.impl("scatter_add_records", &scatter_add_records);
  m.impl("apply_records_sgd", &apply_records_sgd);
  m.impl("arena_digest", &arena_digest);
// ... 62 lines not shown
```

gaussiank_sgd_amd/ops/csrc/kernels/bn_act.hip:

```cpp
#include <hip/hip_runtime.h>

#include <atomic>

#include "common.h"
#include "gk_kernels.h"

namespace gk {
namespace {

constexpr size_t kFinStateFlagsOffset = 16;

__device__ __forceinline__ float bf16_to_f32(uint16_t h) { return __uint_as_float(((uint32_t)h) << 16); }
__device__ __forceinline__ uint16_t f32_to_bf16(float f);
__device__ __forceinline__ float round_to_bf16(float f) { return bf16_to_f32(f32_to_bf16(f)); }
__device__ __forceinline__ void store_elem(float* p, float v) { *p = v; }
__device__ __forceinline__ void store_elem(uint16_t* p, float v) { *p = f32_to_bf16(v); }

__device__ __forceinline__ uint16_t f32_to_bf16(float f) {
  uint32_t u = __float_as_uint(f);
  if ((u & 0x7f800000u) == 0x7f800000u && (u & 0x7fffffu)) return (uint16_t)((u >> 16) | 0x40);
  u += 0x7fffu + ((u >> 16) & 1u);
  return (uint16_t)(u >> 16);
}

// ... 1105 lines not shown
}

void bn_act_backward(BnShape sh, const void* dy, const void* dy2, const uint8_t* mask, const void* x, void* dx,
                     void* dres, const BnBwdStats& bs, float* ws, int relu, void* fin_state, hipStream_t s) {
  with_elem(sh.elem_bytes, [&](auto t) {
    using T = decltype(t);
    with_dy((const T*)dy, (const T*)dy2, mask, relu, [&](auto src) {
      if (!(dy2 && dres)) return bn_backward_src<T>(src, (const T*)x, (T*)dx, (T*)dres, sh, bs, ws, fin_state, s);
      const Geo g = make_geo<T>(sh.M, sh.C, g_bn_blocks);
      const WsParts p = ws_parts(ws, g, sh.C);
      launch_reduce<T, true>(src, (const T*)x, sh, g, bs, p, s, (T*)dres);
      bn_backward_dz<T>((const T*)dres, (const T*)x, (T*)dx, sh, g, bs, bwd_fin(bs, p), fin_state, s);
    });
  });
}

void bn_act_backward_pre(BnShape sh, const void* dz, const void* x, void* dx, const BnBwdStats& bs, BnPartials part,
                         void* fin_state, hipStream_t s) {
  with_elem(sh.elem_bytes, [&](auto t) {
    using T = decltype(t);
    const Geo g = make_geo<T>(sh.M, sh.C, g_bn_blocks);
    bn_backward_dz<T>((const T*)dz, (const T*)x, (T*)dx, sh, g, bs, bwd_fin(bs, part, true), fin_state, s);
  });
}

void bn_bwd_finalize_lazy(BnShape sh, BnPartials part, int center, const BnBwdStats& bs, BnLazyOut lazy,
                          hipStream_t s) {
  with_elem(sh.elem_bytes, [&](auto t) {
    using T = decltype(t);
    hipLaunchKernelGGL(bn_bwd_finalize_lazy_kernel<T>, fin_grid(sh.C), dim3(kBlock), 0, s, part.a, part.b, part.gy,
                       sh.C, sh.M, center, bs.w, bs.mean, bs.invstd, bs.dbeta, bs.dgamma, bs.gb_acc, bs.gw_acc,
                       reinterpret_cast<float4*>(lazy.coef), static_cast<T*>(lazy.padz), static_cast<T*>(lazy.padx));
  });
}

void bn_act_backward_lazy(BnShape sh, const void* dy, const void* dy2, const uint8_t* mask, const void* x, void* dz,
                          const BnBwdStats& bs, float* ws, int relu, BnLazyOut lazy, hipStream_t s) {
  with_elem(sh.elem_bytes, [&](auto t) {
    using T = decltype(t);
    const Geo g = make_geo<T>(sh.M, sh.C, g_bn_blocks);
    const WsParts p = ws_parts(ws, g, sh.C);
    with_dy((const T*)dy, (const T*)dy2, mask, relu,
            [&](auto src) { launch_reduce<T, true>(src, (const T*)x, sh, g, bs, p, s, (T*)dz); });
    bn_bwd_finalize_lazy(sh, p, 0, bs, lazy, s);
  });
}


template <typename T>
__global__ __launch_bounds__(kBlock) void bn_lazy_apply_kernel(const T* __restrict__ dz, const T* __restrict__ x,
                                                               T* __restrict__ dx, int64_t M, int C, Geo g,
                                                               const float4* __restrict__ coef) {
  constexpr int V = Vec<T>::N;
  const int tc = threadIdx.x % g.tpr;
  const int lane_r = threadIdx.x / g.tpr;
  const int c0 = blockIdx.x * g.ct + tc * V;
  float4 cf[V];
#pragma unroll
  for (int i = 0; i < V; ++i) cf[i] = coef[c0 + i];
  const int64_t r0 = (int64_t)blockIdx.y * g.rows_per_block;
  int64_t r1 = r0 + g.rows_per_block;
  if (r1 > M) r1 = M;
  for (int64_t r = lane_r < g.rl ? r0 + lane_r : r1; r < r1; r += g.rl) {
    float d[V], xv[V], o[V];
    Vec<T>::load(dz + r * C + c0, d);
    Vec<T>::load(x + r * C + c0, xv);
#pragma unroll
    for (int i = 0; i < V; ++i) o[i] = cf[i].x * ((d[i] - cf[i].y) - (xv[i] - cf[i].z) * cf[i].w);
    Vec<T>::store(dx + r * C + c0, o);
  }
}

void bn_lazy_apply(BnShape sh, const void* dz, const void* x, void* dx, const float* coef, hipStream_t s) {
  with_elem(sh.elem_bytes, [&](auto t) {
    using T = decltype(t);
    const Geo g = make_geo<T>(sh.M, sh.C, g_bn_blocks);
    hipLaunchKernelGGL(bn_lazy_apply_kernel<T>, grid_of(g), dim3(kBlock), 0, s, (const T*)dz, (const T*)x, (T*)dx, sh.M,
                       sh.C, g, reinterpret_cast<const float4*>(coef));
  });
}

void bn_act_backward_pre_dual(BnShape sh, const void* dz, const void* x, void* dx, const BnBwdStats& bs,
                              BnPartials part, const void* x2, void* dx2, const BnBwdStats& bs2, float* ws2,
                              hipStream_t s) {
  with_elem(sh.elem_bytes, [&](auto t) {
    using T = decltype(t);
    using Src = DyPlain<T, false, false>;
    const Geo g = make_geo<T>(sh.M, sh.C, g_bn_blocks);
    const WsParts p2 = ws_parts(ws2, g, sh.C);
    const Src src{(const T*)dz, nullptr, nullptr};
    launch_reduce<T>(src, (const T*)x2, sh, g, bs2, p2, s);
    launch_bwd_finalize(bwd_fin(bs2, p2), sh.C, s);
    launch_bwd_finalize(bwd_fin(bs, part, true), sh.C, s);
    const BwdDual<T> d2{(const T*)x2, (T*)dx2, bs2.w, bs2.mean, bs2.invstd, bs2.dbeta, bs2.dgamma};
    hipLaunchKernelGGL((bn_bwd_apply_kernel<T, Src, false, false, kBnUnroll, true>), grid_of(g), dim3(kBlock), 0, s,
                       src, (const T*)x, (T*)dx, (T*)nullptr, sh.M, sh.C, g, bs.w, bs.mean, bs.invstd, bs.dbeta,
                       bs.dgamma, FinSync{}, BwdFin{}, d2);
  });
}

void bn_relu_pool_forward(BnShape sh, PoolGeo pg, const void* x, void* y, uint8_t* amax, const BnFwdStats& st,
                          BnPartials pre, float* ws, hipStream_t s) {
  with_elem(sh.elem_bytes, [&](auto t) {
    using T = decltype(t);
    launch_finalize(fwd_fin(st, stats_partials(sh, (const T*)x, pre, ws, s)), sh.M, sh.C, s);
    launch_pool<T>((const T*)x, (T*)y, amax, sh, pg, st.scale, st.shift, s);
  });
}

void bn_relu_pool_backward(BnShape sh, PoolGeo pg, const void* dy, const void* dy2, const uint8_t* amax,
                           const void* x, void* dx, const BnBwdStats& bs, float* ws, hipStream_t s) {
  with_elem(sh.elem_bytes, [&](auto t) {
    using T = decltype(t);
    if (dy2)
      bn_pool_backward_tw<T, true>((const T*)dy, (const T*)dy2, amax, (const T*)x, (T*)dx, sh, pg, bs, ws, s);
    else
      bn_pool_backward_tw<T, false>((const T*)dy, (const T*)dy2, amax, (const T*)x, (T*)dx, sh, pg, bs, ws, s);
  });
}

}
```

gaussiank_sgd_amd/ops/csrc/kernels/gemm.hip:

```cpp
#include "common.h"
#include "gemm_cfg.h"
#include "gemm_units.h"
#include "mfma_util.h"

namespace gk {

static int nt_unit(cfg::Unit unit, bool gather, GK_NT_UNIT_ARGS) {
  switch (unit) {
    case cfg::Unit::b16: return gather ? nt_b16_gat(GK_NT_UNIT_PASS) : nt_b16_row(GK_NT_UNIT_PASS);
    case cfg::Unit::x6: return gather ? nt_x6_gat(GK_NT_UNIT_PASS) : nt_x6_row(GK_NT_UNIT_PASS);
    case cfg::Unit::x62:
      if (gather)
        return nt_x62_gat(static_cast<const float*>(A), static_cast<const float*>(B), static_cast<float*>(C), M, N, K,
                          w, max_blocks, geo, stats, stats_ld, stats_rows, bb, stream);
      return nt_x62_row(static_cast<const float*>(A), lda, static_cast<const float*>(B), ldb, static_cast<float*>(C),
                        ldc, M, N, K, w, max_blocks, geo.bias, stats, stats_ld, stats_rows, bb, geo.b3, stream);
    default: return gather ? nt_f32_gat(GK_NT_UNIT_PASS) : nt_f32_row(GK_NT_UNIT_PASS);
  }
}

__global__ __launch_bounds__(256) void split3_rows_kernel(const float* __restrict__ src, int64_t ld,
                                                          uint16_t* __restrict__ dst, int64_t R, int S) {
  const int64_t g8 = S / 8;
  const int64_t t = (int64_t)blockIdx.x * 256 + threadIdx.x;
// ... 26 lines not shown
                                                               int64_t rows_per_block, BnBwd bb) {
  const int q = threadIdx.x & 63, rl = threadIdx.x >> 6;
  const int n = (blockIdx.y * 64 + q) * 4;
  const bool colok = n < N;
  const int64_t r0 = (int64_t)blockIdx.x * rows_per_block;
  const int64_t r1 = r0 + rows_per_block < M ? r0 + rows_per_block : M;
  const int64_t plane = M * (int64_t)N;
  const float* hp = static_cast<const float*>(bb.h);
  const float* d2p = static_cast<const float*>(bb.dy2);
  f32x4 b = f32x4{0.f, 0.f, 0.f, 0.f};
  if (bias && colok) b = *reinterpret_cast<const f32x4*>(bias + n);
  float ps[4] = {0.f, 0.f, 0.f, 0.f}, pq[4] = {0.f, 0.f, 0.f, 0.f};
  if (colok) {
    for (int64_t m = r0 + rl; m < r1; m += 4) {
      const float* src = ws + m * N + n;
      f32x4 v = *reinterpret_cast<const f32x4*>(src);
      for (int z = 1; z < S; ++z) v += *reinterpret_cast<const f32x4*>(src + z * plane);
      v += b;
      if (hp) {
        const f32x4 hv = *reinterpret_cast<const f32x4*>(hp + m * ldc + n);
        const f32x4 d2 = d2p ? *reinterpret_cast<const f32x4*>(d2p + m * ldc + n) : f32x4{0.f, 0.f, 0.f, 0.f};
        const uint32_t bits = bb.mask ? (uint32_t)bb.mask[m * (N >> 2) + (n >> 2)] : 0xfu;
#pragma unroll
        for (int r = 0; r < 4; ++r) {
          const float dz = (bits >> r) & 1u ? v[r] + d2[r] : 0.f;
          v[r] = dz;
          ps[r] += dz;
          pq[r] = fmaf(dz, hv[r], pq[r]);
        }
      } else if (stats) {
#pragma unroll
        for (int r = 0; r < 4; ++r) {
          ps[r] += v[r];
          pq[r] = fmaf(v[r], v[r], pq[r]);
        }
      }
      *reinterpret_cast<f32x4*>(C + m * ldc + n) = v;
    }
  }
  if (!stats) return;
  __shared__ float red[2][4][256];
#pragma unroll
  for (int r = 0; r < 4; ++r) {
    red[0][rl][q * 4 + r] = ps[r];
    red[1][rl][q * 4 + r] = pq[r];
  }
  __syncthreads();
  const int c = threadIdx.x;
  const int nc = blockIdx.y * 256 + c;
  if (nc < N) {
    const float sa = (red[0][0][c] + red[0][1][c]) + (red[0][2][c] + red[0][3][c]);
    const float sb = (red[1][0][c] + red[1][1][c]) + (red[1][2][c] + red[1][3][c]);
    stats[(int64_t)blockIdx.x * N + nc] = sa;
    stats[stats_ld + (int64_t)blockIdx.x * N + nc] = sb;
  }
}

int splitk_reduce(const float* ws, int S, int64_t M, int N, float* C, int64_t ldc, const float* bias, float* stats,
                  int stats_rows, const BnBwdArgs* bn, hipStream_t stream) {
  const BnBwd bb = bn ? BnBwd{bn->h, bn->dy2, bn->mask} : BnBwd{};
  const int ny = (N + 255) / 256;
  int64_t gx = 1024 / ny;
  const int64_t rmax = (M + 3) / 4;
  if (gx > rmax) gx = rmax;
  if (stats && gx > stats_rows) gx = stats_rows;
  if (gx < 1) gx = 1;
  const int64_t rpb = (M + gx - 1) / gx;
  gx = (M + rpb - 1) / rpb;
  hipLaunchKernelGGL(nt_splitk_reduce_kernel, dim3((unsigned)gx, (unsigned)ny), dim3(256), 0, stream, ws, S, M, N, C,
                     ldc, bias, stats, (int64_t)stats_rows * N, rpb, bb);
  return (int)gx;
}

static int nt_run(bool f32, bool gather, const void* A, int64_t lda, const void* B, int64_t ldb, void* C, int64_t ldc,
                  int64_t M, int N, int K, int cfg_word, int max_blocks, const ConvGeo& g, float* stats, int stats_rows,
                  const BnBwdArgs* bn, const LazyArgs* lazy, float* splitk_ws, hipStream_t stream) {
  const cfg::NtWord w = cfg::NtWord::decode(cfg_word);
  if (!f32) lazy = nullptr;
  const int64_t x_elems = gather ? M / ((int64_t)g.OH * g.OW) * g.H * g.W * g.C : 0;
  const cfg::NtPlan p = cfg::nt_plan(w, f32, gather, lazy != nullptr, g.b3 != nullptr, g.RH != 0, splitk_ws != nullptr, K,
                                     g.C, x_elems);
  if (p.status < 0) return p.status;
  if (bn && bn->OW > 0 && (gather || p.unit != cfg::Unit::x62 || p.planes > 1)) return cfg::kCompactDy2;
  if (p.planes > 1) {
    ConvGeo gz = g;
    gz.bias = nullptr;
    gz.b3 = nullptr;
    gz.KZ = p.planes;
    const int r = nt_unit(p.unit, gather, A, lda, B, ldb, splitk_ws, N, M, N, K / p.planes, w, max_blocks, gz, nullptr, 0,
                          0, BnBwd{}, nullptr, stream);
    if (r < 0) return r;
    return splitk_reduce(splitk_ws, p.planes, M, N, static_cast<float*>(C), ldc, g.bias, stats, stats_rows, bn, stream);
  }
  BnBwd bb = bn ? BnBwd{bn->h, bn->dy2, bn->mask, bn->H, bn->W, bn->OH, bn->OW} : BnBwd{};
  if (bb.OW > 0) {
    if (M >= ((int64_t)1 << 31) || M % ((int64_t)bb.H * bb.W) != 0) return cfg::kCompactDy2;
    magic_u32((uint32_t)(bb.H * bb.W), &bb.mg_hw, &bb.sh_hw);
    magic_u32((uint32_t)bb.W, &bb.mg_w, &bb.sh_w);
  }
  return nt_unit(p.unit, gather, A, lda, B, ldb, C, ldc, M, N, K, w, max_blocks, g, stats, (int64_t)stats_rows * N,
                 stats_rows, bb, lazy, stream);
}

int gemm_nt(const void* A, int64_t lda, const void* B, int64_t ldb, void* C, int64_t ldc, int64_t M, int N, int K,
            bool f32, int cfg, int max_blocks, float* stats, int stats_rows, const float* bias, const BnBwdArgs* bn,
            const LazyArgs* lazy, hipStream_t stream, float* splitk_ws, const void* b3) {
  ConvGeo g{};
  g.bias = bias;
  g.b3 = static_cast<const uint16_t*>(b3);
  return nt_run(f32, false, A, lda, B, ldb, C, ldc, M, N, K, cfg, max_blocks, g, stats, stats_rows, bn, lazy, splitk_ws,
                stream);
}

int conv_nt(const void* X, const void* zero, int H, int W, int C, int OH, int OW, int S, int P, int KH, int KW,
            const void* B, void* Y, int64_t M, int N, bool f32, int cfg, int max_blocks, float* stats, int stats_rows,
            const float* bias, const BnBwdArgs* bn, const LazyArgs* lazy, hipStream_t stream, float* splitk_ws, const void* b3) {
  ConvGeo g{zero, H, W, C, OH, OW, S, P, KW, bias};
  g.b3 = static_cast<const uint16_t*>(b3);
  const int K = KH * KW * C;
  return nt_run(f32, true, X, C, B, K, Y, N, M, N, K, cfg, max_blocks, g, stats, stats_rows, bn, lazy, splitk_ws, stream);
}

int conv_nt_remap(const void* X, int64_t ldx, const void* zero, int H, int W, int C, int OH, int OW, int KH, int KW,
                  const void* B, void* Y, int64_t M, int N, int RH, int RW, int RA, int RB, int RZ, bool f32, int cfg,
                  int max_blocks, const LazyArgs* lazy, hipStream_t stream) {
  ConvGeo g{zero, H, W, C, OH, OW, 1, 0, KW, nullptr, RH, RW, RA, RB, RZ};
  const int K = KH * KW * C;
  const bool gather = KH * KW != 1;
  return nt_run(f32, gather, X, gather ? C : ldx, B, K, Y, N, M, N, K, cfg, max_blocks, g, nullptr, 0, nullptr, lazy,
                nullptr, stream);
}

static int tn_run(bool f32, bool gather, const void* G, int64_t ldg, const void* X, int64_t ldx, float* W, int64_t ldw,
                  int64_t M, int N, int K, int cfg_word, int splits, const ConvGeo& geo, const LazyArgs* lazy,
                  hipStream_t stream) {
  if (!f32) {
    tn_unit_b16(gather, G, ldg, X, ldx, W, ldw, M, N, K, cfg::TnWord::decode(cfg_word), splits, geo, stream);
    return 0;
  }
  const cfg::TnF32Word w = cfg::TnF32Word::decode(cfg_word);
  const cfg::TnPlan p = cfg::tn_plan(w, gather, lazy != nullptr);
  if (p.status < 0) return p.status;
  auto g = static_cast<const float*>(G);
  auto x = static_cast<const float*>(X);
  if (p.unit == cfg::Unit::x62) tn_x62_row(g, ldg, x, ldx, W, ldw, M, N, K, w, splits, stream);
  else if (p.unit == cfg::Unit::x6) tn_unit_x6(gather, g, ldg, x, ldx, W, ldw, M, N, K, w, splits, geo, lazy, stream);
  else tn_unit_f32(gather, g, ldg, x, ldx, W, ldw, M, N, K, w, splits, geo, lazy, stream);
  return 0;
}

int gemm_tn_acc(const void* G, int64_t ldg, const void* X, int64_t ldx, float* W, int64_t ldw, int64_t M, int N,
                 int K, bool f32, int cfg, int splits, const LazyArgs* lazy, hipStream_t stream) {
  return tn_run(f32, false, G, ldg, X, ldx, W, ldw, M, N, K, cfg, splits, ConvGeo{}, lazy, stream);
}

int conv_tn_acc(const void* G, const void* X, const void* zero, int H, int W_, int C, int OH, int OW, int S, int P,
                 int KH, int KW, float* Wout, int64_t M, int N, bool f32, int cfg, int splits, const LazyArgs* lazy,
                 hipStream_t stream) {
  ConvGeo g{zero, H, W_, C, OH, OW, S, P, KW, nullptr};
  const int K = KH * KW * C;
  return tn_run(f32, true, G, N, X, C, Wout, K, M, N, K, cfg, splits, g, lazy, stream);
}

}
```

gaussiank_sgd_amd/ops/csrc/kernels/gemm_cfg.h:

```cpp
#pragma once

#include <cstdint>

namespace gk {
namespace cfg {

enum Status : int {
  kDoesNotFit = -1,
  kRowGemmsOnly = -2,
  kCompactDy2 = -3,
};

inline int family_of(int cfg) {
  const int f = (cfg / 100000) % 10;
  return f >= 1 && f <= 3 ? f : 0;
}

struct NtWord {
  int tile;
  int panel;
  int stages;
  bool wave32;
  int planes;
  int family;
  static NtWord decode(int cfg) {
    const int p = (cfg / 10) % 10, s = (cfg / 100) % 10;
    return NtWord{cfg % 10,           p == 0 ? -1 : (p == 1 ? 1 : 0), s == 1 ? 2 : (s == 2 ? 4 : 3),
                  (cfg / 1000) % 10 == 1, (cfg / 10000) % 10,             family_of(cfg)};
  }
};

struct TnWord {
  int tile;
  int stages;
  static TnWord decode(int cfg) { return TnWord{cfg % 10 + 10 * ((cfg / 100) % 10), (cfg / 10) % 10 == 2 ? 3 : 2}; }
};

struct TnF32Word {
  int tile;
  int stages;
  int family;
  static TnF32Word decode(int cfg) {
    return TnF32Word{(cfg % 100000) % 10, (cfg / 10) % 10 != 1 ? 3 : 2, family_of(cfg)};
  }
};

struct NtSel {
  int wm, wn, msb;
  bool bnb, lz;
  int panel, stages;
};
constexpr int nt_key(int wm, int wn, int msb, bool bnb, bool lz) {
  return (((wm * 8 + wn) * 16 + msb) * 2 + (bnb ? 1 : 0)) * 2 + (lz ? 1 : 0);
}

inline NtSel nt_select(const NtWord& w, int N, bool f32, bool x6, bool bn, bool lazy) {
  static const int bn64[8] = {64, 64, 128, 256, 128, 256, 128, 256};
  int t = w.tile;
  if (t <= 0) t = N % 256 == 0 ? 3 : (N % 128 == 0 ? 2 : 1);
  if (t > 7 || N % bn64[t] != 0) t = 1;
  NtSel s{4, 1, 4, bn, f32 && lazy, w.panel, w.stages};
  if (f32 && w.wave32 && !lazy) {
    static const int bn32[8] = {64, 64, 128, 64, 256, 128, 256, 128};
    static const int wm32[8] = {4, 4, 2, 2, 1, 4, 2, 1}, wn32[8] = {1, 1, 2, 1, 4, 2, 4, 2};
    t = w.tile;
    if (t <= 0 || t > 7 || N % bn32[t] != 0) t = 1;
    s.wm = wm32[t], s.wn = wn32[t], s.msb = 2;
    return s;
  }
  if (bn || s.lz) {
    static const int wm[8] = {4, 4, 4, 2, 2, 2, 2, 2}, wn[8] = {1, 1, 2, 4, 2, 4, 2, 4};
    s.wm = wm[t], s.wn = wn[t];
    return s;
  }
  static const int wm[8] = {4, 4, 4, 2, 2, 2, 2, 1}, wn[8] = {1, 1, 2, 4, 2, 4, 2, 4};
  s.wm = wm[t], s.wn = wn[t];
  if (t >= 5 && (!f32 || x6)) s.msb = 8;
  return s;
}

struct TnSel {
  int wn, wk, ws, stages;
};
constexpr int tn_key(int wn, int wk, int ws) { return (wn * 8 + wk) * 8 + ws; }

inline TnSel tn_select(const TnWord& w, int N, int K) {
  static const int bn[13] = {64, 64, 128, 64, 128, 256, 64, 128, 64, 256, 64, 128, 256};
  static const int bk[13] = {64, 64, 64, 128, 128, 64, 256, 128, 64, 128, 64, 256, 256};
  static const int wn[13] = {1, 1, 2, 1, 2, 4, 1, 2, 1, 4, 1, 2, 4}, wk[13] = {1, 1, 1, 2, 2, 1, 4, 2, 1, 2, 1, 4, 4};
  static const int ws[13] = {4, 4, 2, 2, 1, 1, 1, 2, 2, 1, 4, 1, 1};
  int t = w.tile;
  if (t <= 0) {
    const bool n2 = N % 128 == 0, k2 = K % 128 == 0;
// ... 90 lines not shown
```

gaussiank_sgd_amd/ops/csrc/kernels/gemm_nt_x62.h:

```cpp
#pragma once

#include "gemm_common.h"

namespace gk {
namespace {

template <int WM, int WN>
struct X62Cfg {
  static constexpr int NW = WM * WN;
  static constexpr int THREADS = 64 * NW;
  static constexpr int BM = 64 * WM;
  static constexpr int BN = 64 * WN;
  static constexpr int PA = BM * 64;
  static constexpr int PB = BN * 64;
  static constexpr int STAGE = 3 * (PA + PB);
  static constexpr int LDS = 2 * STAGE;
  static constexpr int PRA = BM * 4 / THREADS;
  static constexpr int PRB = BN * 4 / THREADS;
  static_assert(PRA >= 1 && PRB >= 1 && (BM * 4) % THREADS == 0 && (BN * 4) % THREADS == 0, "pieces per thread");
  static_assert(LDS <= 160 * 1024, "LDS");
};

template <int WM, int WN, bool BNB, int NPF = 1, bool GATHER = false, bool P3 = false, bool D2C = false>
__global__ void __launch_bounds__(64 * WM * WN) __attribute__((amdgpu_waves_per_eu(1)))
gemm_nt_x62_kernel(const float* __restrict__ A, int64_t lda, const float* __restrict__ B, int64_t ldb,
                   float* __restrict__ C, int64_t ldc, int64_t M, int K, const float* __restrict__ bias,
                   float* __restrict__ stats, int64_t stats_ld, BnBwd bb, ConvGeo geo) {
  using Cfg = X62Cfg<WM, WN>;
  extern __shared__ __attribute__((aligned(16))) char smem[];
  int bx, by;
  xcd_remap2(bx, by);
  const int tid = threadIdx.x;
  const int lane = tid & 63;
  const int wave = __builtin_amdgcn_readfirstlane(tid >> 6);
  const int wm = wave / WN, wn = wave % WN;
  const int fr = lane & 15, fq = lane >> 4;
  const int n0 = by * Cfg::BN;
  const int Ntot = (int)gridDim.y * Cfg::BN;
  const int64_t mtiles = (M + Cfg::BM - 1) / Cfg::BM;
  const int nk = K / 32;
  const int64_t my_tiles = bx < mtiles ? (mtiles - 1 - bx) / gridDim.x + 1 : 0;
  const int T_ = (int)(my_tiles * nk);
  if (T_ == 0) {
    if (stats)
      for (int c = tid; c < Cfg::BN; c += Cfg::THREADS) {
        stats[(int64_t)bx * Ntot + n0 + c] = 0.f;
        stats[stats_ld + (int64_t)bx * Ntot + n0 + c] = 0.f;
      }
    return;
  }

  f32x4 ra[NPF][Cfg::PRA][2], rb[NPF][P3 ? 1 : Cfg::PRB][2];
  u32x4 rb3[NPF][P3 ? Cfg::PRB : 1][3];
  const uint16_t* lpb3[P3 ? Cfg::PRB : 1];
  int64_t l_mt = bx;
  int l_ks = 0;
  const float* lpa[GATHER ? 1 : Cfg::PRA];
  const float* lpb[Cfg::PRB];
  int l_kh = 0, l_kw = 0, l_c0 = 0;
  uint32_t okhw[GATHER ? Cfg::PRA : 1];
  int32_t aoff[GATHER ? Cfg::PRA : 1];
  auto set_a_rows = [&]() __attribute__((always_inline)) {
    const int64_t m0 = l_mt * Cfg::BM;
#pragma unroll
    for (int p = 0; p < Cfg::PRA; ++p) {
      const int cid = tid + Cfg::THREADS * p;
      int64_t gr = m0 + (cid >> 2);
      gr = gr < M ? gr : M - 1;
      if constexpr (GATHER) {
        const uint32_t ohw = (uint32_t)(geo.OH * geo.OW);
        const uint32_t mu = (uint32_t)gr;
        const uint32_t n = mu / ohw, rem = mu - n * ohw;
        const uint32_t oh = rem / (uint32_t)geo.OW, ow = rem - oh * (uint32_t)geo.OW;
        const int ih0 = (int)oh * geo.S - geo.P, iw0 = (int)ow * geo.S - geo.P;
        uint32_t bh = 0u, bw = 0u;
#pragma unroll
        for (int t = 0; t < kMaxTaps; ++t) {
          bh |= (uint32_t)((unsigned)(ih0 + t) < (unsigned)geo.H) << t;
          bw |= (uint32_t)((unsigned)(iw0 + t) < (unsigned)geo.W) << t;
        }
        okhw[p] = bh | (bw << 8);
        aoff[p] = (((int)n * geo.H + ih0) * geo.W + iw0) * geo.C + (cid & 3) * 8;
      } else {
        lpa[p] = A + gr * lda + (cid & 3) * 8;
      }
    }
  };
  set_a_rows();
#pragma unroll
  for (int p = 0; p < Cfg::PRB; ++p) {
    const int cid = tid + Cfg::THREADS * p;
    if constexpr (P3) lpb3[p] = geo.b3 + (int64_t)(n0 + (cid >> 2)) * (3 * K) + (cid & 3) * 8;
    else lpb[p] = B + (int64_t)(n0 + (cid >> 2)) * ldb + (cid & 3) * 8;
  }
  const float* zrow = static_cast<const float*>(geo.zero);
  auto issue_loads = [&](auto SET) __attribute__((always_inline)) {
    constexpr int q = decltype(SET)::value;
    const int64_t toff = GATHER ? (int64_t)(l_kh * geo.W + l_kw) * geo.C + l_c0 : 0;
#pragma unroll
    for (int p = 0; p < Cfg::PRA; ++p) {
      const float* src;
      if constexpr (GATHER) {
        const bool ok = ((okhw[p] >> l_kh) & (okhw[p] >> (8 + l_kw)) & 1u) != 0u;
        src = ok ? A + ((int64_t)aoff[p] + toff) : zrow;
      } else {
        src = lpa[p];
        lpa[p] += 32;
      }
      ra[q][p][0] = *reinterpret_cast<const f32x4*>(src);
      ra[q][p][1] = *reinterpret_cast<const f32x4*>(src + 4);
    }
#pragma unroll
    for (int p = 0; p < Cfg::PRB; ++p) {
      if constexpr (P3) {
#pragma unroll
        for (int pl = 0; pl < 3; ++pl) rb3[q][p][pl] = *reinterpret_cast<const u32x4*>(lpb3[p] + pl * 32);
        lpb3[p] += 96;
      } else {
        rb[q][p][0] = *reinterpret_cast<const f32x4*>(lpb[p]);
        rb[q][p][1] = *reinterpret_cast<const f32x4*>(lpb[p] + 4);
        lpb[p] += 32;
      }
    }
    if constexpr (GATHER) {
      l_c0 += 32;
      if (l_c0 == geo.C) {
        l_c0 = 0;
        if (++l_kw == geo.KW) {
          l_kw = 0;
          ++l_kh;
        }
      }
    }
    if (++l_ks == nk) {
      l_ks = 0;
      l_kh = l_kw = l_c0 = 0;
      l_mt += gridDim.x;
      set_a_rows();
#pragma unroll
      for (int p = 0; p < Cfg::PRB; ++p) {
        if constexpr (P3) lpb3[p] -= 3 * K;
        else lpb[p] -= K;
      }
    }
  };
  auto split_write = [&](int buf, auto SET, int pc = -1) __attribute__((always_inline)) {
    constexpr int q = decltype(SET)::value;
    char* st = smem + buf * Cfg::STAGE;
#pragma unroll
    for (int p = 0; p < Cfg::PRA; ++p) {
      if (pc >= 0 && pc != p) continue;
      const int cid = tid + Cfg::THREADS * p;
      const int r = cid >> 2;
      bf16x8 h, m, l;
      split3x8(ra[q][p][0], ra[q][p][1], h, m, l);
      const int off = r * 64 + (((cid & 3) ^ x62_swz(r)) << 4);
      *reinterpret_cast<bf16x8*>(st + off) = h;
      *reinterpret_cast<bf16x8*>(st + Cfg::PA + off) = m;
      *reinterpret_cast<bf16x8*>(st + 2 * Cfg::PA + off) = l;
    }
    char* sb = st + 3 * Cfg::PA;
#pragma unroll
    for (int p = 0; p < Cfg::PRB; ++p) {
      if (pc >= 0 && pc != Cfg::PRA + p) continue;
      const int cid = tid + Cfg::THREADS * p;
      const int r = cid >> 2;
      const int off = r * 64 + (((cid & 3) ^ x62_swz(r)) << 4);
      if constexpr (P3) {
        *reinterpret_cast<u32x4*>(sb + off) = rb3[q][p][0];
        *reinterpret_cast<u32x4*>(sb + Cfg::PB + off) = rb3[q][p][1];
        *reinterpret_cast<u32x4*>(sb + 2 * Cfg::PB + off) = rb3[q][p][2];
      } else {
        bf16x8 h, m, l;
        split3x8(rb[q][p][0], rb[q][p][1], h, m, l);
        *reinterpret_cast<bf16x8*>(sb + off) = h;
        *reinterpret_cast<bf16x8*>(sb + Cfg::PB + off) = m;
        *reinterpret_cast<bf16x8*>(sb + 2 * Cfg::PB + off) = l;
      }
    }
  };

  f32x4 acc[4][4];
#pragma unroll
  for (int a = 0; a < 4; ++a)
#pragma unroll
    for (int b = 0; b < 4; ++b) acc[a][b] = f32x4{0.f, 0.f, 0.f, 0.f};
  float ssum[4][4], ssq[4][4], bia[BNB ? 1 : 4][4];
#pragma unroll
  for (int a = 0; a < 4; ++a)
#pragma unroll
    for (int b = 0; b < 4; ++b) {
      ssum[a][b] = ssq[a][b] = 0.f;
      if constexpr (!BNB) bia[a][b] = bias ? bias[n0 + wn * 64 + a * 16 + fq * 4 + b] : 0.f;
    }

  auto epilogue = [&](int64_t mt) __attribute__((always_inline)) {
    const int64_t mbase = mt * Cfg::BM;
    constexpr int EH = BNB ? 1 : 4;
#pragma unroll
    for (int ms = 0; ms < 4; ++ms) {
      const int64_t m = mbase + wm * 64 + ms * 16 + fr;
      const bool live = m < M;
#pragma unroll
      for (int nh = 0; nh < 4; nh += EH) {
      f32x4 ehv[EH], ed2[EH];
      uint32_t ebits[EH];
      if constexpr (BNB) {
#pragma unroll
        for (int e = 0; e < EH; ++e) {
          ehv[e] = ed2[e] = f32x4{0.f, 0.f, 0.f, 0.f};
          ebits[e] = 0u;
        }
        if (live) {
          int32_t d2row = -1;
          if constexpr (BNB && D2C) {
            const uint32_t mu = (uint32_t)m;
            const uint32_t img = (__umulhi(mu, bb.mg_hw) + mu) >> bb.sh_hw, rem = mu - img * (uint32_t)(bb.H * bb.W);
            const uint32_t ph = (__umulhi(rem, bb.mg_w) + rem) >> bb.sh_w, pw = rem - ph * (uint32_t)bb.W;
            if (((ph | pw) & 1u) == 0u) d2row = (int32_t)((img * (uint32_t)bb.OH + (ph >> 1)) * (uint32_t)bb.OW + (pw >> 1));
          }
#pragma unroll
          for (int e = 0; e < EH; ++e) {
            const int n = n0 + wn * 64 + (nh + e) * 16 + fq * 4;
            ehv[e] = *reinterpret_cast<const f32x4*>(static_cast<const float*>(bb.h) + m * ldc + n);
            if constexpr (D2C) {
              if (d2row >= 0)
                ed2[e] = *reinterpret_cast<const f32x4*>(static_cast<const float*>(bb.dy2) + (int64_t)d2row * ldc + n);
            } else {
              if (bb.dy2) ed2[e] = *reinterpret_cast<const f32x4*>(static_cast<const float*>(bb.dy2) + m * ldc + n);
            }
            ebits[e] = bb.mask ? (uint32_t)bb.mask[m * (Ntot >> 2) + (n >> 2)] : 0xfu;
          }
        }
      }
#pragma unroll
      for (int e = 0; e < EH; ++e) {
        const int ns = nh + e;
        const int n = n0 + wn * 64 + ns * 16 + fq * 4;
        f32x4 v = acc[ms][ns];
        acc[ms][ns] = f32x4{0.f, 0.f, 0.f, 0.f};
        if constexpr (!BNB) {
#pragma unroll
          for (int r = 0; r < 4; ++r) v[r] += bia[ns][r];
        }
        if constexpr (BNB) {
#pragma unroll
          for (int r = 0; r < 4; ++r) {
            const float dz = (ebits[e] >> r) & 1u ? v[r] + ed2[e][r] : 0.f;
            v[r] = dz;
            ssum[ns][r] += dz;
            ssq[ns][r] = fmaf(dz, ehv[e][r], ssq[ns][r]);
          }
        } else {
          if (stats && live) {
#pragma unroll
            for (int r = 0; r < 4; ++r) {
              ssum[ns][r] += v[r];
              ssq[ns][r] = fmaf(v[r], v[r], ssq[ns][r]);
            }
          }
        }
        if (live) *reinterpret_cast<f32x4*>(C + m * ldc + n) = v;
      }
      }
    }
  };

  using I0 = std::integral_constant<int, 0>;
  using I1 = std::integral_constant<int, (NPF > 1 ? 1 : 0)>;
  issue_loads(I0{});
  split_write(0, I0{});
  if (T_ > 1) issue_loads(I1{});
  if (NPF > 1 && T_ > 2) issue_loads(I0{});
  __syncthreads();
  int ks = 0;
  int64_t mt = bx;
  auto slice = [&](int t, auto PAR) __attribute__((always_inline)) {
    constexpr int par = decltype(PAR)::value;
    using SN = std::integral_constant<int, (NPF > 1 ? (par ^ 1) : 0)>;
    const int cur = par;
    const char* st = smem + cur * Cfg::STAGE;
    const char* pa = st;
    const char* pb = st + 3 * Cfg::PA;
    auto frag = [&](const char* plane, int row) __attribute__((always_inline)) -> bf16x8 {
      return *reinterpret_cast<const bf16x8*>(plane + row * 64 + ((fq ^ x62_swz(row)) << 4));
    };
    bf16x8 bh[4], bm[4], bl[4];
#pragma unroll
    for (int ns = 0; ns < 4; ++ns) {
      const int row = wn * 64 + ns * 16 + fr;
      bh[ns] = frag(pb, row);
      bm[ns] = frag(pb + Cfg::PB, row);
      bl[ns] = frag(pb + 2 * Cfg::PB, row);
    }
    constexpr int NPC = Cfg::PRA + Cfg::PRB;
#pragma unroll
    for (int ms = 0; ms < 4; ++ms) {
      const int row = wm * 64 + ms * 16 + fr;
      const bf16x8 ah = frag(pa, row), am = frag(pa + Cfg::PA, row), al = frag(pa + 2 * Cfg::PA, row);
#pragma unroll
      for (int ns = 0; ns < 4; ++ns) {
        f32x4 c = acc[ms][ns];
        c = __builtin_amdgcn_mfma_f32_16x16x32_bf16(bl[ns], ah, c, 0, 0, 0);
        c = __builtin_amdgcn_mfma_f32_16x16x32_bf16(bh[ns], al, c, 0, 0, 0);
        c = __builtin_amdgcn_mfma_f32_16x16x32_bf16(bm[ns], am, c, 0, 0, 0);
        c = __builtin_amdgcn_mfma_f32_16x16x32_bf16(bm[ns], ah, c, 0, 0, 0);
        c = __builtin_amdgcn_mfma_f32_16x16x32_bf16(bh[ns], am, c, 0, 0, 0);
        acc[ms][ns] = __builtin_amdgcn_mfma_f32_16x16x32_bf16(bh[ns], ah, c, 0, 0, 0);
        const int gstep = 4 * ms + ns;
        if (gstep >= 1 && gstep <= NPC) split_write(cur ^ 1, SN{}, gstep - 1);
        if (gstep == NPC + 1) issue_loads(SN{});
        __builtin_amdgcn_sched_barrier(0);
      }
    }
    if (++ks == nk) {
      ks = 0;
      epilogue(mt);
      mt += gridDim.x;
    }
    __syncthreads();
  };
  for (int t = 0; t < T_; t += 2) {
    slice(t, I0{});
    if (t + 1 < T_) slice(t + 1, std::integral_constant<int, 1>{});
  }

  if (stats) {
#pragma unroll
    for (int a = 0; a < 4; ++a)
#pragma unroll
      for (int b = 0; b < 4; ++b)
#pragma unroll
        for (int off = 1; off < 16; off <<= 1) {
          ssum[a][b] += __shfl_xor(ssum[a][b], off, 64);
          ssq[a][b] += __shfl_xor(ssq[a][b], off, 64);
        }
    float* red = reinterpret_cast<float*>(smem);
    if (fr == 0) {
#pragma unroll
      for (int a = 0; a < 4; ++a)
#pragma unroll
        for (int b = 0; b < 4; ++b) {
          const int col = wn * 64 + a * 16 + fq * 4 + b;
          red[wm * Cfg::BN + col] = ssum[a][b];
          red[(WM + wm) * Cfg::BN + col] = ssq[a][b];
        }
    }
    __syncthreads();
    for (int c = tid; c < Cfg::BN; c += Cfg::THREADS) {
      float sa = 0.f, sb = 0.f;
#pragma unroll
      for (int w2 = 0; w2 < WM; ++w2) {
        sa += red[w2 * Cfg::BN + c];
        sb += red[(WM + w2) * Cfg::BN + c];
      }
      stats[(int64_t)bx * Ntot + n0 + c] = sa;
      stats[stats_ld + (int64_t)bx * Ntot + n0 + c] = sb;
    }
  }
}

template <int WM, int WN, bool BNB, int NPF, bool GATHER, bool P3 = false, bool D2C = false>
int launch_nt_x62(const float* A, int64_t lda, const float* B, int64_t ldb, float* C, int64_t ldc, int64_t M, int N,
                  int K, int max_blocks, const float* bias, float* stats, int64_t stats_ld, int stats_rows,
                  const BnBwd& bb, const ConvGeo& geo, hipStream_t stream) {
  using Cfg = X62Cfg<WM, WN>;
  const int ntiles = N / Cfg::BN;
  const int64_t mtiles = (M + Cfg::BM - 1) / Cfg::BM;
  const int per_cu = (160 * 1024) / Cfg::LDS > 0 ? (160 * 1024) / Cfg::LDS : 1;
  int64_t gx = ((int64_t)256 * per_cu + ntiles - 1) / ntiles;
  if (max_blocks > 0) gx = max_blocks;
  if (gx < 1) gx = 1;
  if (gx > mtiles) gx = mtiles;
  if (stats && gx > stats_rows) gx = stats_rows;
  static bool attr = [] {
    return hipFuncSetAttribute(reinterpret_cast<const void*>(&gemm_nt_x62_kernel<WM, WN, BNB, NPF, GATHER, P3, D2C>),
                               hipFuncAttributeMaxDynamicSharedMemorySize, 160 * 1024) == hipSuccess;
  }();
  (void)attr;
  hipLaunchKernelGGL((gemm_nt_x62_kernel<WM, WN, BNB, NPF, GATHER, P3, D2C>), dim3((unsigned)gx, (unsigned)ntiles), dim3(Cfg::THREADS),
                     Cfg::LDS, stream, A, lda, B, ldb, C, ldc, M, K, bias, stats, stats_ld, bb, geo);
  return (int)gx;
}

template <bool GATHER>
int nt_x62_dispatch(const float* A, int64_t lda, const float* B, int64_t ldb, float* C, int64_t ldc, int64_t M,
                    int N, int K, const cfg::NtWord& w, int max_blocks, const float* bias, float* stats,
                    int64_t stats_ld, int stats_rows, const BnBwd& bb, const ConvGeo& geo, hipStream_t stream) {
  const cfg::X62NtSel s = cfg::nt_x62_select(w, N, geo.b3 != nullptr, bb.h != nullptr);
#define GK_X62L(WM_, WN_, BNB_, P3_, D2C_)                                                                   \
  launch_nt_x62<WM_, WN_, BNB_, 1, GATHER, P3_, D2C_>(A, lda, B, ldb, C, ldc, M, N, K, max_blocks, bias, stats, \
                                                      stats_ld, stats_rows, bb, geo, stream)
#define GK_X62N(WM_, WN_, P3_)                                             \
  do {                                                                     \
    if constexpr (!GATHER)                                                 \
      if (s.bnb && bb.OW > 0) return GK_X62L(WM_, WN_, true, P3_, true);   \
    return s.bnb ? GK_X62L(WM_, WN_, true, P3_, false) : GK_X62L(WM_, WN_, false, P3_, false); \
  } while (0)
#define GK_X62(WM_, WN_)               \
  case cfg::x62_key(WM_, WN_):         \
    if (s.p3) GK_X62N(WM_, WN_, true); \
    GK_X62N(WM_, WN_, false)
  switch (cfg::x62_key(s.wm, s.wn)) {
    GK_X62(2, 4);
    GK_X62(4, 2);
    GK_X62(1, 4);
    GK_X62(4, 1);
    GK_X62(1, 2);
    GK_X62(2, 1);
    GK_X62(2, 2);
  }
#undef GK_X62
#undef GK_X62N
#undef GK_X62L
  return cfg::kDoesNotFit;
}

}
}
```

gaussiank_sgd_amd/ops/csrc/kernels/gemm_units.h:

```cpp
#pragma once

#include <hip/hip_runtime.h>

#include "gemm_cfg.h"
#include "gk_kernels.h"

namespace gk {

constexpr int kMaxTaps = 4;

struct ConvGeo {
  const void* zero;
  int H, W, C, OH, OW, S, P, KW;
  const float* bias;
  int RH, RW, RA, RB, RZ;
  int KZ;
  const uint16_t* b3;
};

struct BnBwd {
  const void* h;
  const void* dy2;
  const uint8_t* mask;
  int H, W, OH, OW;
  uint32_t mg_hw, sh_hw, mg_w, sh_w;
};

inline void magic_u32(uint32_t d, uint32_t* mg, uint32_t* sh) {
  uint32_t s = 0;
  while (((uint64_t)1 << s) < d) ++s;
  *sh = s;
  *mg = (uint32_t)(((((uint64_t)1 << s) - d) << 32) / d + 1);
}

struct LazyA {
  const void* x;
  const float* coef;
  const void* padz;
  const void* padx;
  int C;
};

#define GK_NT_UNIT_ARGS                                                                                  \
  const void *A, int64_t lda, const void *B, int64_t ldb, void *C, int64_t ldc, int64_t M, int N, int K, \
      const cfg::NtWord &w, int max_blocks, const ConvGeo &geo, float *stats, int64_t stats_ld,         \
      int stats_rows, const BnBwd &bb, const LazyArgs *lza, hipStream_t stream
#define GK_NT_UNIT_PASS A, lda, B, ldb, C, ldc, M, N, K, w, max_blocks, geo, stats, stats_ld, stats_rows, bb, lza, stream
int nt_b16_row(GK_NT_UNIT_ARGS);
int nt_b16_gat(GK_NT_UNIT_ARGS);
int nt_f32_row(GK_NT_UNIT_ARGS);
int nt_f32_gat(GK_NT_UNIT_ARGS);
int nt_x6_row(GK_NT_UNIT_ARGS);
int nt_x6_gat(GK_NT_UNIT_ARGS);
int nt_x62_row(const float* A, int64_t lda, const float* B, int64_t ldb, float* C, int64_t ldc, int64_t M, int N, int K,
               const cfg::NtWord& w, int max_blocks, const float* bias, float* stats, int64_t stats_ld, int stats_rows,
               const BnBwd& bb, const uint16_t* b3, hipStream_t stream);
int nt_x62_gat(const float* A, const float* B, float* C, int64_t M, int N, int K, const cfg::NtWord& w, int max_blocks,
               const ConvGeo& geo, float* stats, int64_t stats_ld, int stats_rows, const BnBwd& bb,
               hipStream_t stream);
void tn_x62_row(const float* G, int64_t ldg, const float* X, int64_t ldx, float* W, int64_t ldw, int64_t M, int N,
                int K, const cfg::TnF32Word& w, int splits, hipStream_t stream);
void tn_unit_x6(bool gather, const float* G, int64_t ldg, const float* X, int64_t ldx, float* W, int64_t ldw,
                int64_t M, int N, int K, const cfg::TnF32Word& w, int splits, const ConvGeo& geo, const LazyArgs* lza,
                hipStream_t stream);
void tn_unit_b16(bool gather, const void* G, int64_t ldg, const void* X, int64_t ldx, float* W, int64_t ldw, int64_t M,
                 int N, int K, const cfg::TnWord& w, int splits, const ConvGeo& geo, hipStream_t stream);
void tn_unit_f32(bool gather, const float* G, int64_t ldg, const float* X, int64_t ldx, float* W, int64_t ldw,
                 int64_t M, int N, int K, const cfg::TnF32Word& w, int splits, const ConvGeo& geo, const LazyArgs* lza,
                 hipStream_t stream);

}
```

gaussiank_sgd_amd/ops/csrc/kernels/gk_kernels.h:

```cpp
#pragma once

#include <hip/hip_runtime.h>
#include <stddef.h>
#include <stdint.h>

namespace gk {

enum Mode : int {
  kModeGaussian = 0,
  kModeRedSync = 1,
  kModeRedSyncTrim = 2,
  kModeTopK = 3,
  kModeRandomK = 4,
  kModeThreshold = 5,
  kModeDGC = 6,
  kModeGaussianCal = 7,
};

constexpr int kCalFallback = 16;
constexpr int kOverflowExact = 17;

constexpr int kMaxCand = 16;
constexpr int kRecHdr = 4;
constexpr int kMaxCountBlocks = 1024;
// ... 136 lines not shown
void fused_adam(const AdamArgs& a, hipStream_t stream);

struct LambGroup : AdamHyper {
  double trust_clip;
  int adapt;
  int pad0;
};
struct LambArgs : MomentArgs {
  LambGroup groups[kMaxGroups] = {};
  const int32_t* seg_range = nullptr;
  int nseg = 0;
  double* part = nullptr;
  float* trust = nullptr;
  int passes = 7;
};
void fused_lamb(const LambArgs& a, hipStream_t stream);

struct McArgs {
  float* u = nullptr;
  float* g = nullptr;
  const float* w = nullptr;
  const Chunk* chunks = nullptr;
  int nchunks = 0;
  float momentum[kMaxGroups];
  float weight_decay[kMaxGroups];
};
void momentum_correct(const McArgs& a, hipStream_t stream);
void mask_records(float* u, const int32_t* record, int64_t k_cap, hipStream_t stream);

void accum_grad(float* dst, const void* src, int64_t n, int src_bytes, hipStream_t stream);
void cast_bf16(uint16_t* dst, const float* src, int64_t n, hipStream_t stream);

void segmented_sumsq(const float* w, const float* g, const Chunk* chunks, int nchunks, double* out,
                     hipStream_t stream);

struct LarsArgs {
  float* w = nullptr;
  float* m = nullptr;
  const float* g = nullptr;
  const Chunk* chunks = nullptr;
  int nchunks = 0;
  const double* seg_sumsq = nullptr;
  float lr[kMaxGroups], momentum[kMaxGroups], weight_decay[kMaxGroups], eeta[kMaxGroups],
      epsilon[kMaxGroups];
  int ngroups = 0;
};
void fused_lars(const LarsArgs& a, hipStream_t stream);

void clip_grad_norm(float* g, int64_t n, float max_norm, double* ws, float* coef_out,
                    float* norm_out, hipStream_t stream);

struct BnShape { int64_t M; int C; int elem_bytes; };
struct BnPartials { const float* a; const float* b; int gy; };
struct BnFwdStats {
  const float* w; const float* b;
  float eps, momentum;
  float* run_mean; float* run_var; float* save_mean; float* save_invstd; float* scale; float* shift;
  int64_t* nbt;
};
struct BnBwdStats {
  const float* w; const float* mean; const float* invstd;
  float* dgamma; float* dbeta; float* gw_acc; float* gb_acc;
};
struct BnResidual { const void* res; const float* rscale; const float* rshift; };
struct BnLazyOut { float* coef; void* padz; void* padx; };
size_t bn_workspace_floats(int64_t M, int C, int elem_bytes);
size_t bn_fin_state_bytes(int C);
bool bn_supported(int C, int elem_bytes);
void bn_set_blocks(int blocks);
size_t bn_mask_bytes(int64_t M, int C, int elem_bytes);
void bn_stats_partials(BnShape sh, const void* x, float* ws, hipStream_t stream);
void bn_act_forward(BnShape sh, const void* x, BnResidual res, void* y, uint8_t* mask, const BnFwdStats& st,
                    BnPartials pre, float* ws, int relu, void* fin_state, hipStream_t stream);
void bn_act_finalize(BnShape sh, const void* x, const BnFwdStats& st, BnPartials pre, float* ws, hipStream_t stream);
void bn_bwd_finalize_lazy(BnShape sh, BnPartials part, int center, const BnBwdStats& bs, BnLazyOut lazy,
                          hipStream_t stream);
void bn_act_backward_lazy(BnShape sh, const void* dy, const void* dy2, const uint8_t* mask, const void* x, void* dz,
                          const BnBwdStats& bs, float* ws, int relu, BnLazyOut lazy, hipStream_t stream);
void bn_lazy_apply(BnShape sh, const void* dz, const void* x, void* dx, const float* coef, hipStream_t stream);
void bn_act_backward_pre(BnShape sh, const void* dz, const void* x, void* dx, const BnBwdStats& bs, BnPartials part,
                         void* fin_state, hipStream_t stream);
void bn_act_backward_pre_dual(BnShape sh, const void* dz, const void* x, void* dx, const BnBwdStats& bs,
                              BnPartials part, const void* x2, void* dx2, const BnBwdStats& bs2, float* ws2,
                              hipStream_t stream);
void bn_act_backward(BnShape sh, const void* dy, const void* dy2, const uint8_t* mask, const void* x, void* dx,
                     void* dres, const BnBwdStats& bs, float* ws, int relu, void* fin_state, hipStream_t stream);

struct PoolGeo {
  int H, W, OH, OW, k, s, p;
};
void bn_relu_pool_forward(BnShape sh, PoolGeo pg, const void* x, void* y, uint8_t* amax, const BnFwdStats& st,
                          BnPartials pre, float* ws, hipStream_t stream);
void bn_relu_pool_backward(BnShape sh, PoolGeo pg, const void* dy, const void* dy2, const uint8_t* amax,
                           const void* x, void* dx, const BnBwdStats& bs, float* ws, hipStream_t stream);

bool gemm_supported(int64_t N, int64_t K);
struct BnBwdArgs {
  const void* h;
  const void* dy2;
  const uint8_t* mask;
  int H, W, OH, OW;
};
struct LazyArgs {
  const void* x;
  const float* coef;
  const void* padz;
  const void* padx;
  int C;
};
int gemm_nt(const void* A, int64_t lda, const void* B, int64_t ldb, void* C, int64_t ldc, int64_t M, int N, int K,
            bool f32, int cfg, int max_blocks, float* stats, int stats_rows, const float* bias, const BnBwdArgs* bn,
            const LazyArgs* lazy, hipStream_t stream, float* splitk_ws = nullptr, const void* b3 = nullptr);
int splitk_reduce(const float* ws, int S, int64_t M, int N, float* C, int64_t ldc, const float* bias, float* stats,
                  int stats_rows, const BnBwdArgs* bn, hipStream_t stream);
int gemm_tn_acc(const void* G, int64_t ldg, const void* X, int64_t ldx, float* W, int64_t ldw, int64_t M, int N,
                 int K, bool f32, int cfg, int splits, const LazyArgs* lazy, hipStream_t stream);
int conv_nt(const void* X, const void* zero, int H, int W, int C, int OH, int OW, int S, int P, int KH, int KW,
            const void* B, void* Y, int64_t M, int N, bool f32, int cfg, int max_blocks, float* stats, int stats_rows,
            const float* bias, const BnBwdArgs* bn, const LazyArgs* lazy, hipStream_t stream,
            float* splitk_ws = nullptr, const void* b3 = nullptr);
void split3_rows(const float* src, int64_t ld, void* dst, int64_t R, int S, hipStream_t stream);
int conv_nt_remap(const void* X, int64_t ldx, const void* zero, int H, int W, int C, int OH, int OW, int KH, int KW,
                  const void* B, void* Y, int64_t M, int N, int RH, int RW, int RA, int RB, int RZ, bool f32, int cfg,
                  int max_blocks, const LazyArgs* lazy, hipStream_t stream);
int conv_tn_acc(const void* G, const void* X, const void* zero, int H, int W, int C, int OH, int OW, int S, int P,
                 int KH, int KW, float* Wout, int64_t M, int N, bool f32, int cfg, int splits, const LazyArgs* lazy,
                 hipStream_t stream);
bool stem_f32_supported(int H, int W);
int stem_f32_wgrad_blocks(int N);
int stem_f32x6_wplanes();
int stem_f32x6_forward(const float* x, int N, int H, int W, const float* w, int64_t s0, int64_t s1, int64_t s2,
                       int64_t s3, uint16_t* wp3, float* y, float* stats, int stats_rows, hipStream_t stream);
int stem_f32_forward(const float* x, int N, int H, int W, const float* w, int64_t s0, int64_t s1, int64_t s2,
                     int64_t s3, float* y, float* stats, int stats_rows, hipStream_t stream);
void stem_f32_wgrad(const float* x, const float* dy, int N, int H, int W, float* part, float* out, int64_t s0,
                    int64_t s1, int64_t s2, int64_t s3, bool x6, hipStream_t stream);
void wino_weights(const float* w, float* u, int Co, int Ci, int flip, hipStream_t stream);
enum PrepKind : int32_t { kPrepWino = 0, kPrepWinoFlip = 1, kPrepT32 = 2, kPrepT16 = 3, kPrepWinoX6 = 4,
                          kPrepWinoX6Flip = 5 };
struct PrepDesc {
  const void* src;
  void* dst;
  int64_t ld_in, ld_out;
  int64_t block_begin;
  int32_t kind, R, S, tiles_s;
};
static_assert(sizeof(PrepDesc) == 56, "PrepDesc layout is packed by ops/weight_prep.py");
int64_t weight_prep_blocks(int kind, int R, int S);
int weight_prep_max_descs();
void weight_prep(const PrepDesc* descs, int ndesc, int64_t total_blocks, hipStream_t stream);
int wino_conv(const float* x, const float* u, float* y, int N, int H, int W, int Ci, int Co, int max_blocks,
              float* stats, int stats_rows, const BnBwdArgs* bn, hipStream_t stream, int splits = 1,
              float* split_ws = nullptr);
void wino_x6_weights(const float* w, uint16_t* u3, int Co, int Ci, int flip, hipStream_t stream);
int wino_x6_conv(const float* x, const uint16_t* u3, float* y, int N, int H, int W, int Ci, int Co, int max_blocks,
                 float* stats, int stats_rows, const BnBwdArgs* bn, hipStream_t stream);
int wino_wgrad_splits(int N, int H, int W, int C, int K, int splits);
void wino_wgrad(const float* x, const float* dy, float* part, float* out, int N, int H, int W, int C, int K,
                int splits, hipStream_t stream);

bool stem_supported(int H, int W);
void stem_pack_weight(const float* w, int64_t s0, int64_t s1, int64_t s2, int64_t s3, uint16_t* wp,
                      hipStream_t stream);
int stem_forward(const void* x, bool x_f32, int N, int H, int W, const uint16_t* wp, uint16_t* y, float* stats,
                 int stats_rows, hipStream_t stream);
int stem_wgrad_blocks(int N, int H, int W);
void stem_wgrad(const void* x, bool x_f32, int N, int H, int W, const uint16_t* dy, float* part, float* out,
                int64_t s0, int64_t s1, int64_t s2, int64_t s3, hipStream_t stream);

bool wgrad3_supported(int H, int W, int C, int K);
int64_t wgrad3_ws_floats(int N, int H, int W, int C, int K);
void wgrad3_acc(const void* dy, const void* x, const void* zero, int N, int H, int W, int C, int K, float* part,
                float* out, int64_t s0, int64_t s1, int64_t s2, int64_t s3, hipStream_t stream);

bool attn_supported(int T, int D);
bool attn_f32_supported(int T, int D);
void attn_f32_fwd(const float* qkv, float* out, float* lse, int B, int T, int H, float p, uint32_t seed,
                  const uint32_t* seed_dev, const uint32_t* key_bits, bool causal, hipStream_t stream);
void attn_f32_bwd(const float* qkv, const float* out, const float* dout, const float* lse, float* delta, float* dqkv,
                  int B, int T, int H, float p, uint32_t seed, const uint32_t* seed_dev, const uint32_t* key_bits,
                  bool causal, hipStream_t stream);
void attn_fwd(const void* qkv, void* out, float* lse, int B, int T, int H, float p, uint32_t seed,
              const uint32_t* seed_dev, const uint32_t* key_bits, void* out_lo, bool causal, hipStream_t stream);
void attn_bwd(const void* qkv, const void* out, const void* dout, const float* lse, float* delta, void* dqkv, int B,
// ... 58 lines not shown
```

Before: 5057 images/s.

## Fuse downsample BN's second reduction into the 1x1 dgrad GEMM epilogue

When the BN output feeds a downsample branch whose BN input has the same shape, the 1x1 dgrad GEMM epilogue now also accumulates sum(dz*h2) for the second BN into a third stats plane. It uses DPP row reductions and a small extra LDS region. The dual backward then skips its separate reduce kernel over dz and x2, saving one full read pass of two activations. The cost is an extra h2 load per epilogue element, more LDS per block, and new template instances with their own autotune key. It is limited to fp32 with bf16x6 register-staged row GEMMs and no split-K.

```diff
diff --git a/gaussiank_sgd_amd/ops/bn.py b/gaussiank_sgd_amd/ops/bn.py
--- a/gaussiank_sgd_amd/ops/bn.py
+++ b/gaussiank_sgd_amd/ops/bn.py
@@ -30,10 +30,10 @@
 
 class BnLink:
 
-    __slots__ = ("h", "mask", "twin", "dy2", "dz", "part", "dy2c", "geo")
+    __slots__ = ("h", "mask", "twin", "dy2", "dz", "part", "dy2c", "geo", "h2", "part2")
 
     def __init__(self):
-        self.h = self.mask = self.dy2 = self.dz = self.part = self.dy2c = self.geo = None
+        self.h = self.mask = self.dy2 = self.dz = self.part = self.dy2c = self.geo = self.h2 = self.part2 = None
         self.twin = False
 
     def ready(self) -> bool:
@@ -50,7 +50,7 @@
         return full
 
     def clear(self) -> None:
-        self.h = self.mask = self.dy2 = self.dz = self.part = self.dy2c = self.geo = None
+        self.h = self.mask = self.dy2 = self.dz = self.part = self.dy2c = self.geo = self.h2 = self.part2 = None
 
 
 class ProducerLink:
@@ -125,6 +125,8 @@
         ctx.plink = plink
         if link is not None:
             link.h, link.mask, link.twin = x, mask, bool(twin)
+            if dlink is not None and dlink.x.shape == x.shape and dlink.x.dtype == x.dtype:
+                link.h2 = dlink.x
         return (y, y.view_as(y)) if twin else y
 
     @staticmethod
@@ -139,6 +141,7 @@
             if dz is None or dz.data_ptr() != link.dz.data_ptr():
                 raise RuntimeError("BNAct bwd_link: the linked output had another consumer")
             part, rows = link.part
+            part2 = link.part2
             link.clear()
             g = torch.empty(2, x.shape[1], dtype=torch.float32, device=x.device)
             if lazy:
@@ -151,13 +154,14 @@
                 x2 = dlink.x
                 dx2 = torch.empty_like(x2, memory_format=_CL)
                 g2 = torch.empty(2, x2.shape[1], dtype=torch.float32, device=x.device)
-                ws2 = torch.empty(int(_ops().bn_workspace_floats(x2.numel() // x2.shape[1], x2.shape[1],
-                                                                 x2.element_size())),
-                                  dtype=torch.float32, device=x.device)
+                ws2 = None if part2 is not None else \
+                    torch.empty(int(_ops().bn_workspace_floats(x2.numel() // x2.shape[1], x2.shape[1],
+                                                               x2.element_size())),
+                                dtype=torch.float32, device=x.device)
                 gw2, gb2 = dlink.direct if dlink.direct is not None else (None, None)
                 _ops().bn_act_backward_pre_dual(dz, x, dx, weight, mean, invstd, g[0], g[1], part, rows, gw, gb, x2,
                                                 dx2, dlink.weight, dlink.mean, dlink.invstd, g2[0], g2[1], ws2, gw2,
-                                                gb2)
+                                                gb2, part2)
                 dlink.dz, dlink.dx, dlink.g = dz, dx2, g2
             else:
                 dx = torch.empty_like(x, memory_format=_CL)
diff --git a/gaussiank_sgd_amd/ops/conv1x1.py b/gaussiank_sgd_amd/ops/conv1x1.py
--- a/gaussiank_sgd_amd/ops/conv1x1.py
+++ b/gaussiank_sgd_amd/ops/conv1x1.py
@@ -235,6 +235,8 @@
 def _dgrad_bn(dy: torch.Tensor, w: torch.Tensor, x_shape, s: int, link, lz=None, plink=None,
               wp: bool = False) -> torch.Tensor:
     N, C, H, W, K, k, p, OH, OW = _geom(x_shape, w, s)
+    if lz is None and _h2_fusable(link, w, dy.dtype):
+        return _dgrad_bn2(dy, w, x_shape, link, wp=wp)
     kw = _lz_kw(lz, rows=(k == 1)) if lz is not None else {}
     g = _g()
     M = N * H * W
@@ -273,6 +275,33 @@
     else:
         rows = run(ch[1], ch[2])
     link.part = (st, int(rows))
+    link.dz = dz
+    return dz
+
+
+def _h2_fusable(link, w: torch.Tensor, dt: torch.dtype) -> bool:
+    h2 = getattr(link, "h2", None)
+    return (h2 is not None and w.shape[2] == 1 and dt == torch.float32 and f32_matmul() == "bf16x6" and
+            h2.dtype == dt and h2.shape == link.h.shape and os.environ.get("GKSGD_BN_LINK_DS2", "1") != "0")
+
+
+def _dgrad_bn2(dy: torch.Tensor, w: torch.Tensor, x_shape, link, wp: bool = False) -> torch.Tensor:
+    N, C, H, W, K, k, p, OH, OW = _geom(x_shape, w, 1)
+    g = _g()
+    M = N * H * W
+    dt = dy.dtype
+    dz = torch.empty(x_shape, dtype=dt, device=dy.device, memory_format=_CL)
+    st = torch.empty(3, min(1280, (M + 63) // 64), C, dtype=torch.float32, device=dy.device)
+    DY, DZ, H1, H2 = _rows(dy), _rows(dz), _rows(link.h), _rows(link.h2)
+    D2 = _rows(link.dy2) if link.dy2 is not None else None
+    mask = link.mask
+    Wt = _lazy(lambda: weight_prep.transposed_1x1(w, wp))
+    run = lambda c, mb: g.gemm_nt(DY, Wt(), DZ, c, mb, st, None, H1, D2, mask, bn_h2=H2)
+    cands = autotune.hip_cands(run, product(autotune.nt_x62_cfgs(), autotune.NT_GRIDS))
+    ch = autotune.pick(("dgrad_bn2", N, C, H, W, K, D2 is not None) + autotune.dkey(dt), cands)
+    rows = run(ch[1], ch[2])
+    link.part = (st[:2], int(rows))
+    link.part2 = st[2]
     link.dz = dz
     return dz
 
diff --git a/gaussiank_sgd_amd/ops/csrc/bindings.cpp b/gaussiank_sgd_amd/ops/csrc/bindings.cpp
--- a/gaussiank_sgd_amd/ops/csrc/bindings.cpp
+++ b/gaussiank_sgd_amd/ops/csrc/bindings.cpp
@@ -617,16 +617,26 @@
                               at::Tensor invstd, at::Tensor dgamma, at::Tensor dbeta, at::Tensor part, int64_t rows,
                               OptTensor gw_acc, OptTensor gb_acc, at::Tensor x2, at::Tensor dx2, OptTensor w2,
                               at::Tensor mean2, at::Tensor invstd2, at::Tensor dgamma2, at::Tensor dbeta2,
-                              at::Tensor ws2, OptTensor gw2_acc, OptTensor gb2_acc) {
+                              OptTensor ws2, OptTensor gw2_acc, OptTensor gb2_acc, OptTensor part_ds) {
   const gk::BnShape sh = bn_shape(x);
   check_same(x, {&dz, &dx, &x2, &dx2}, "dz / dx / x2 / dx2");
   const gk::BnBwdStats bs = bwd_stats(w, mean, invstd, dgamma, dbeta, gw_acc, gb_acc, sh.C);
   const gk::BnBwdStats bs2 = bwd_stats(w2, mean2, invstd2, dgamma2, dbeta2, gw2_acc, gb2_acc, sh.C);
   const gk::BnPartials p = partials(part, rows, sh.C, "part");
-  float* wp2 = check_ws(ws2, sh);
+  gk::BnPartials p2{};
+  float* wp2 = nullptr;
+  if (has(part_ds)) {
+    TORCH_CHECK(part_ds->is_cuda() && part_ds->scalar_type() == at::kFloat && part_ds->is_contiguous() &&
+                    part_ds->dim() == 2 && part_ds->size(0) >= rows && part_ds->size(1) == sh.C,
+                "part_ds must be fp32 [rows, C] partials with at least the used rows");
+    p2 = gk::BnPartials{p.a, part_ds->data_ptr<float>(), p.gy};
+  } else {
+    TORCH_CHECK(has(ws2), "ws2: needed without part_ds");
+    wp2 = check_ws(*ws2, sh);
+  }
   c10::DeviceGuard guard(x.device());
   gk::bn_act_backward_pre_dual(sh, dz.data_ptr(), x.data_ptr(), dx.data_ptr(), bs, p, x2.data_ptr(), dx2.data_ptr(),
-                               bs2, wp2, cur_stream(x));
+                               bs2, wp2, p2, cur_stream(x));
 }
 
 gk::BnLazyOut lazy_out(const at::Tensor& x, int C, const at::Tensor& coef, const at::Tensor& padz,
@@ -904,15 +914,15 @@
   TORCH_CHECK(reinterpret_cast<uintptr_t>(t.data_ptr()) % 16 == 0, name, " must be 16-byte aligned");
 }
 
-float* stats_ptr(const c10::optional<at::Tensor>& st, int64_t N, int* rows) {
+float* stats_ptr(const c10::optional<at::Tensor>& st, int64_t N, int* rows, int64_t planes = 2) {
   if (!st.has_value()) {
     *rows = 0;
     return nullptr;
   }
   const at::Tensor& t = *st;
-  TORCH_CHECK(t.is_cuda() && t.scalar_type() == at::kFloat && t.is_contiguous() && t.dim() == 3 && t.size(0) == 2 &&
-                  t.size(2) == N && t.size(1) > 0,
-              "stats must be a contiguous fp32 [2, rows, N] GPU tensor");
+  TORCH_CHECK(t.is_cuda() && t.scalar_type() == at::kFloat && t.is_contiguous() && t.dim() == 3 &&
+                  t.size(0) == planes && t.size(2) == N && t.size(1) > 0,
+              "stats must be a contiguous fp32 [2, rows, N] GPU tensor ([3, rows, N] with bn_h2)");
   *rows = (int)t.size(1);
   return t.data_ptr<float>();
 }
@@ -1059,10 +1069,12 @@
 bool bn_bwd_args(const c10::optional<at::Tensor>& h, const c10::optional<at::Tensor>& dy2,
                  const c10::optional<at::Tensor>& mask, int64_t M, int64_t N,
                  int64_t ldc, bool has_stats, at::ScalarType dt, gk::BnBwdArgs* out,
-                 c10::OptionalArrayRef<int64_t> dy2_geo = c10::nullopt) {
+                 c10::OptionalArrayRef<int64_t> dy2_geo = c10::nullopt,
+                 const c10::optional<at::Tensor>& h2 = c10::nullopt) {
   const bool compact = dy2_geo.has_value();
+  const bool second = h2.has_value() && h2->defined();
   if (!h.has_value() || !h->defined()) {
-    TORCH_CHECK(!compact, "bn_dy2_geo needs the BN-backward epilogue operands");
+    TORCH_CHECK(!compact && !second, "bn_dy2_geo / bn_h2 need the BN-backward epilogue operands");
     return false;
   }
   TORCH_CHECK(has_stats, "BN-backward epilogue needs the stats partials buffer");
@@ -1074,6 +1086,12 @@
   };
   rows_ok(*h, "bn h");
   out->h = h->data_ptr();
+  out->h2 = nullptr;
+  if (second) {
+    TORCH_CHECK(dt == at::kFloat && !compact, "bn_h2: fp32, not together with a compact bn_dy2");
+    rows_ok(*h2, "bn h2");
+    out->h2 = h2->data_ptr();
+  }
   out->dy2 = nullptr;
   out->H = out->W = out->OH = out->OW = 0;
   if (compact) {
@@ -1147,6 +1165,9 @@
                 ": the register-staged bf16x6 kernels (cfg digit 200000/300000) take plain row GEMMs only");
     TORCH_CHECK(r != gk::cfg::kCompactDy2, op,
                 ": a compact bn_dy2 takes one register-staged bf16x6 row GEMM (cfg digit 200000/300000, no split-K)");
+    TORCH_CHECK(r != gk::cfg::kSecondH, op,
+                ": bn_h2 takes one register-staged bf16x6 row GEMM (cfg digit 200000/300000, no split-K, no compact "
+                "bn_dy2)");
     TORCH_CHECK(r >= 0, op, ": the lazy operand's coefficient table does not fit this tile configuration");
     return r;
   }
@@ -1156,7 +1177,7 @@
                 c10::optional<at::Tensor> stats, c10::optional<at::Tensor> bias, c10::optional<at::Tensor> bn_h,
                 c10::optional<at::Tensor> bn_dy2, c10::optional<at::Tensor> bn_mask, c10::optional<at::Tensor> lz_x, c10::optional<at::Tensor> lz_coef,
                 c10::optional<at::Tensor> lz_padz, c10::optional<at::Tensor> lz_padx,
-                c10::OptionalArrayRef<int64_t> bn_dy2_geo) {
+                c10::OptionalArrayRef<int64_t> bn_dy2_geo, c10::optional<at::Tensor> bn_h2) {
   check_rows(A, "A", A);
   check_rows(B, "B", A);
   check_rows(C, "C", A);
@@ -1165,10 +1186,10 @@
   TORCH_CHECK(gk::gemm_supported(N, K), "gemm_nt: N and K must be multiples of 64");
   TORCH_CHECK(M > 0, "gemm_nt: empty M");
   int rows = 0;
-  float* sp = stats_ptr(stats, N, &rows);
+  float* sp = stats_ptr(stats, N, &rows, bn_h2.has_value() && bn_h2->defined() ? 3 : 2);
   gk::BnBwdArgs bn{};
   const bool has_bn = bn_bwd_args(bn_h, bn_dy2, bn_mask, M, N, C.stride(0), sp != nullptr, C.scalar_type(), &bn,
-                                  bn_dy2_geo);
+                                  bn_dy2_geo, bn_h2);
   TORCH_CHECK(!has_bn || !bias.has_value() || !bias->defined(), "gemm_nt: bias and BN epilogue are exclusive");
   gk::LazyArgs lz{};
   const bool has_lz = lazy_args(lz_x, lz_coef, lz_padz, lz_padx, A, K, &lz);
@@ -2003,7 +2024,7 @@
   m.def("gemm_supported(int N, int K) -> bool", &gemm_supported);
   m.def("gemm_nt(Tensor A, Tensor B, Tensor(a!) C, int cfg=0, int max_blocks=0, Tensor(b!)? stats=None, "
         "Tensor? bias=None, Tensor? bn_h=None, Tensor? bn_dy2=None, Tensor? bn_mask=None, Tensor? lz_x=None, Tensor? lz_coef=None, Tensor? lz_padz=None, Tensor? lz_padx=None, "
-        "int[]? bn_dy2_geo=None) -> int");
+        "int[]? bn_dy2_geo=None, Tensor? bn_h2=None) -> int");
   m.def("gemm_tn_acc(Tensor G, Tensor X, Tensor(a!) W, int cfg=0, int splits=0, Tensor? lz_x=None, Tensor? lz_coef=None, Tensor? lz_padz=None, Tensor? lz_padx=None) -> ()");
   m.def("conv_nt(Tensor x, Tensor w, Tensor(a!) y, Tensor zero, int stride, int pad, int cfg=0, int max_blocks=0, "
         "Tensor(b!)? stats=None, Tensor? bias=None, Tensor? bn_h=None, Tensor? bn_dy2=None, Tensor? bn_mask=None, "
@@ -2048,7 +2069,7 @@
       "bn_act_backward_pre_dual(Tensor dz, Tensor x, Tensor(a!) dx, Tensor? w, Tensor mean, Tensor invstd, "
       "Tensor(b!) dgamma, Tensor(c!) dbeta, Tensor part, int rows, Tensor(d!)? gw_acc, Tensor(e!)? gb_acc, Tensor x2, "
       "Tensor(f!) dx2, Tensor? w2, Tensor mean2, Tensor invstd2, Tensor(g!) dgamma2, Tensor(h!) dbeta2, "
-      "Tensor(i!) ws2, Tensor(j!)? gw2_acc, Tensor(k!)? gb2_acc) -> ()");
+      "Tensor(i!)? ws2, Tensor(j!)? gw2_acc, Tensor(k!)? gb2_acc, Tensor? part_ds=None) -> ()");
   m.def("bn_act_backward_pre(Tensor dz, Tensor x, Tensor(a!) dx, Tensor? w, Tensor mean, Tensor invstd, "
         "Tensor(b!) dgamma, Tensor(c!) dbeta, Tensor part, int rows, Tensor(d!)? gw_acc=None, "
         "Tensor(e!)? gb_acc=None, Tensor(f!)? fin=None) -> ()");
diff --git a/gaussiank_sgd_amd/ops/csrc/kernels/bn_act.hip b/gaussiank_sgd_amd/ops/csrc/kernels/bn_act.hip
--- a/gaussiank_sgd_amd/ops/csrc/kernels/bn_act.hip
+++ b/gaussiank_sgd_amd/ops/csrc/kernels/bn_act.hip
@@ -1211,15 +1211,19 @@
 
 void bn_act_backward_pre_dual(BnShape sh, const void* dz, const void* x, void* dx, const BnBwdStats& bs,
                               BnPartials part, const void* x2, void* dx2, const BnBwdStats& bs2, float* ws2,
-                              hipStream_t s) {
+                              BnPartials part2, hipStream_t s) {
   with_elem(sh.elem_bytes, [&](auto t) {
     using T = decltype(t);
     using Src = DyPlain<T, false, false>;
     const Geo g = make_geo<T>(sh.M, sh.C, g_bn_blocks);
-    const WsParts p2 = ws_parts(ws2, g, sh.C);
     const Src src{(const T*)dz, nullptr, nullptr};
-    launch_reduce<T>(src, (const T*)x2, sh, g, bs2, p2, s);
-    launch_bwd_finalize(bwd_fin(bs2, p2), sh.C, s);
+    if (part2.a) {
+      launch_bwd_finalize(bwd_fin(bs2, part2, true), sh.C, s);
+    } else {
+      const WsParts p2 = ws_parts(ws2, g, sh.C);
+      launch_reduce<T>(src, (const T*)x2, sh, g, bs2, p2, s);
+      launch_bwd_finalize(bwd_fin(bs2, p2), sh.C, s);
+    }
     launch_bwd_finalize(bwd_fin(bs, part, true), sh.C, s);
     const BwdDual<T> d2{(const T*)x2, (T*)dx2, bs2.w, bs2.mean, bs2.invstd, bs2.dbeta, bs2.dgamma};
     hipLaunchKernelGGL((bn_bwd_apply_kernel<T, Src, false, false, kBnUnroll, true>), grid_of(g), dim3(kBlock), 0, s,
diff --git a/gaussiank_sgd_amd/ops/csrc/kernels/gemm.hip b/gaussiank_sgd_amd/ops/csrc/kernels/gemm.hip
--- a/gaussiank_sgd_amd/ops/csrc/kernels/gemm.hip
+++ b/gaussiank_sgd_amd/ops/csrc/kernels/gemm.hip
@@ -132,6 +132,7 @@
                                      g.C, x_elems);
   if (p.status < 0) return p.status;
   if (bn && bn->OW > 0 && (gather || p.unit != cfg::Unit::x62 || p.planes > 1)) return cfg::kCompactDy2;
+  if (bn && bn->h2 && (gather || p.unit != cfg::Unit::x62 || p.planes > 1 || bn->OW > 0)) return cfg::kSecondH;
   if (p.planes > 1) {
     ConvGeo gz = g;
     gz.bias = nullptr;
@@ -143,6 +144,7 @@
     return splitk_reduce(splitk_ws, p.planes, M, N, static_cast<float*>(C), ldc, g.bias, stats, stats_rows, bn, stream);
   }
   BnBwd bb = bn ? BnBwd{bn->h, bn->dy2, bn->mask, bn->H, bn->W, bn->OH, bn->OW} : BnBwd{};
+  bb.h2 = bn ? bn->h2 : nullptr;
   if (bb.OW > 0) {
     if (M >= ((int64_t)1 << 31) || M % ((int64_t)bb.H * bb.W) != 0) return cfg::kCompactDy2;
     magic_u32((uint32_t)(bb.H * bb.W), &bb.mg_hw, &bb.sh_hw);
diff --git a/gaussiank_sgd_amd/ops/csrc/kernels/gemm_cfg.h b/gaussiank_sgd_amd/ops/csrc/kernels/gemm_cfg.h
--- a/gaussiank_sgd_amd/ops/csrc/kernels/gemm_cfg.h
+++ b/gaussiank_sgd_amd/ops/csrc/kernels/gemm_cfg.h
@@ -9,6 +9,7 @@
   kDoesNotFit = -1,
   kRowGemmsOnly = -2,
   kCompactDy2 = -3,
+  kSecondH = -4,
 };
 
 inline int family_of(int cfg) {
diff --git a/gaussiank_sgd_amd/ops/csrc/kernels/gemm_nt_x62.h b/gaussiank_sgd_amd/ops/csrc/kernels/gemm_nt_x62.h
--- a/gaussiank_sgd_amd/ops/csrc/kernels/gemm_nt_x62.h
+++ b/gaussiank_sgd_amd/ops/csrc/kernels/gemm_nt_x62.h
@@ -18,10 +18,20 @@
   static constexpr int PRA = BM * 4 / THREADS;
   static constexpr int PRB = BN * 4 / THREADS;
   static_assert(PRA >= 1 && PRB >= 1 && (BM * 4) % THREADS == 0 && (BN * 4) % THREADS == 0, "pieces per thread");
-  static_assert(LDS <= 160 * 1024, "LDS");
+  static constexpr int H2LDS = NW * 64 * 4;
+  static_assert(LDS + H2LDS <= 160 * 1024, "LDS");
 };
 
-template <int WM, int WN, bool BNB, int NPF = 1, bool GATHER = false, bool P3 = false, bool D2C = false>
+__device__ __forceinline__ float row16_sum(float v) {
+  v += __builtin_bit_cast(float, __builtin_amdgcn_mov_dpp(__builtin_bit_cast(int, v), 0xB1, 0xF, 0xF, true));
+  v += __builtin_bit_cast(float, __builtin_amdgcn_mov_dpp(__builtin_bit_cast(int, v), 0x4E, 0xF, 0xF, true));
+  v += __builtin_bit_cast(float, __builtin_amdgcn_mov_dpp(__builtin_bit_cast(int, v), 0x141, 0xF, 0xF, true));
+  v += __builtin_bit_cast(float, __builtin_amdgcn_mov_dpp(__builtin_bit_cast(int, v), 0x140, 0xF, 0xF, true));
+  return v;
+}
+
+template <int WM, int WN, bool BNB, int NPF = 1, bool GATHER = false, bool P3 = false, bool D2C = false,
+          bool H2 = false>
 __global__ void __launch_bounds__(64 * WM * WN) __attribute__((amdgpu_waves_per_eu(1)))
 gemm_nt_x62_kernel(const float* __restrict__ A, int64_t lda, const float* __restrict__ B, int64_t ldb,
                    float* __restrict__ C, int64_t ldc, int64_t M, int K, const float* __restrict__ bias,
@@ -46,6 +56,7 @@
       for (int c = tid; c < Cfg::BN; c += Cfg::THREADS) {
         stats[(int64_t)bx * Ntot + n0 + c] = 0.f;
         stats[stats_ld + (int64_t)bx * Ntot + n0 + c] = 0.f;
+        if constexpr (H2) stats[2 * stats_ld + (int64_t)bx * Ntot + n0 + c] = 0.f;
       }
     return;
   }
@@ -186,6 +197,8 @@
 #pragma unroll
     for (int b = 0; b < 4; ++b) acc[a][b] = f32x4{0.f, 0.f, 0.f, 0.f};
   float ssum[4][4], ssq[4][4], bia[BNB ? 1 : 4][4];
+  float* sq2 = reinterpret_cast<float*>(smem + Cfg::LDS) + wave * 64;
+  if constexpr (H2) sq2[lane] = 0.f;
 #pragma unroll
   for (int a = 0; a < 4; ++a)
 #pragma unroll
@@ -203,12 +216,12 @@
       const bool live = m < M;
 #pragma unroll
       for (int nh = 0; nh < 4; nh += EH) {
-      f32x4 ehv[EH], ed2[EH];
+      f32x4 ehv[EH], ed2[EH], eh2[EH];
       uint32_t ebits[EH];
       if constexpr (BNB) {
 #pragma unroll
         for (int e = 0; e < EH; ++e) {
-          ehv[e] = ed2[e] = f32x4{0.f, 0.f, 0.f, 0.f};
+          ehv[e] = ed2[e] = eh2[e] = f32x4{0.f, 0.f, 0.f, 0.f};
           ebits[e] = 0u;
         }
         if (live) {
@@ -223,6 +236,7 @@
           for (int e = 0; e < EH; ++e) {
             const int n = n0 + wn * 64 + (nh + e) * 16 + fq * 4;
             ehv[e] = *reinterpret_cast<const f32x4*>(static_cast<const float*>(bb.h) + m * ldc + n);
+            if constexpr (H2) eh2[e] = *reinterpret_cast<const f32x4*>(static_cast<const float*>(bb.h2) + m * ldc + n);
             if constexpr (D2C) {
               if (d2row >= 0)
                 ed2[e] = *reinterpret_cast<const f32x4*>(static_cast<const float*>(bb.dy2) + (int64_t)d2row * ldc + n);
@@ -250,6 +264,15 @@
             v[r] = dz;
             ssum[ns][r] += dz;
             ssq[ns][r] = fmaf(dz, ehv[e][r], ssq[ns][r]);
+          }
+          if constexpr (H2) {
+            f32x4 p2;
+#pragma unroll
+            for (int r = 0; r < 4; ++r) p2[r] = row16_sum(v[r] * eh2[e][r]);
+            if (fr == 0) {
+              f32x4* slot = reinterpret_cast<f32x4*>(sq2 + ns * 16 + fq * 4);
+              *slot += p2;
+            }
           }
         } else {
           if (stats && live) {
@@ -348,19 +371,21 @@
     }
     __syncthreads();
     for (int c = tid; c < Cfg::BN; c += Cfg::THREADS) {
-      float sa = 0.f, sb = 0.f;
+      float sa = 0.f, sb = 0.f, sc = 0.f;
 #pragma unroll
       for (int w2 = 0; w2 < WM; ++w2) {
         sa += red[w2 * Cfg::BN + c];
         sb += red[(WM + w2) * Cfg::BN + c];
+        if constexpr (H2) sc += reinterpret_cast<const float*>(smem + Cfg::LDS)[(w2 * WN + c / 64) * 64 + c % 64];
       }
       stats[(int64_t)bx * Ntot + n0 + c] = sa;
       stats[stats_ld + (int64_t)bx * Ntot + n0 + c] = sb;
+      if constexpr (H2) stats[2 * stats_ld + (int64_t)bx * Ntot + n0 + c] = sc;
     }
   }
 }
 
-template <int WM, int WN, bool BNB, int NPF, bool GATHER, bool P3 = false, bool D2C = false>
+template <int WM, int WN, bool BNB, int NPF, bool GATHER, bool P3 = false, bool D2C = false, bool H2 = false>
 int launch_nt_x62(const float* A, int64_t lda, const float* B, int64_t ldb, float* C, int64_t ldc, int64_t M, int N,
                   int K, int max_blocks, const float* bias, float* stats, int64_t stats_ld, int stats_rows,
                   const BnBwd& bb, const ConvGeo& geo, hipStream_t stream) {
@@ -374,12 +399,12 @@
   if (gx > mtiles) gx = mtiles;
   if (stats && gx > stats_rows) gx = stats_rows;
   static bool attr = [] {
-    return hipFuncSetAttribute(reinterpret_cast<const void*>(&gemm_nt_x62_kernel<WM, WN, BNB, NPF, GATHER, P3, D2C>),
+    return hipFuncSetAttribute(reinterpret_cast<const void*>(&gemm_nt_x62_kernel<WM, WN, BNB, NPF, GATHER, P3, D2C, H2>),
                                hipFuncAttributeMaxDynamicSharedMemorySize, 160 * 1024) == hipSuccess;
   }();
   (void)attr;
-  hipLaunchKernelGGL((gemm_nt_x62_kernel<WM, WN, BNB, NPF, GATHER, P3, D2C>), dim3((unsigned)gx, (unsigned)ntiles), dim3(Cfg::THREADS),
-                     Cfg::LDS, stream, A, lda, B, ldb, C, ldc, M, K, bias, stats, stats_ld, bb, geo);
+  hipLaunchKernelGGL((gemm_nt_x62_kernel<WM, WN, BNB, NPF, GATHER, P3, D2C, H2>), dim3((unsigned)gx, (unsigned)ntiles), dim3(Cfg::THREADS),
+                     Cfg::LDS + (H2 ? Cfg::H2LDS : 0), stream, A, lda, B, ldb, C, ldc, M, K, bias, stats, stats_ld, bb, geo);
   return (int)gx;
 }
 
@@ -388,14 +413,16 @@
                     int N, int K, const cfg::NtWord& w, int max_blocks, const float* bias, float* stats,
                     int64_t stats_ld, int stats_rows, const BnBwd& bb, const ConvGeo& geo, hipStream_t stream) {
   const cfg::X62NtSel s = cfg::nt_x62_select(w, N, geo.b3 != nullptr, bb.h != nullptr);
-#define GK_X62L(WM_, WN_, BNB_, P3_, D2C_)                                                                   \
-  launch_nt_x62<WM_, WN_, BNB_, 1, GATHER, P3_, D2C_>(A, lda, B, ldb, C, ldc, M, N, K, max_blocks, bias, stats, \
-                                                      stats_ld, stats_rows, bb, geo, stream)
+#define GK_X62L(WM_, WN_, BNB_, P3_, D2C_, H2_)                                                                   \
+  launch_nt_x62<WM_, WN_, BNB_, 1, GATHER, P3_, D2C_, H2_>(A, lda, B, ldb, C, ldc, M, N, K, max_blocks, bias, stats, \
+                                                           stats_ld, stats_rows, bb, geo, stream)
 #define GK_X62N(WM_, WN_, P3_)                                             \
   do {                                                                     \
-    if constexpr (!GATHER)                                                 \
-      if (s.bnb && bb.OW > 0) return GK_X62L(WM_, WN_, true, P3_, true);   \
-    return s.bnb ? GK_X62L(WM_, WN_, true, P3_, false) : GK_X62L(WM_, WN_, false, P3_, false); \
+    if constexpr (!GATHER) {                                               \
+      if (s.bnb && bb.OW > 0) return GK_X62L(WM_, WN_, true, P3_, true, false); \
+      if (s.bnb && bb.h2) return GK_X62L(WM_, WN_, true, P3_, false, true);     \
+    }                                                                      \
+    return s.bnb ? GK_X62L(WM_, WN_, true, P3_, false, false) : GK_X62L(WM_, WN_, false, P3_, false, false); \
   } while (0)
 #define GK_X62(WM_, WN_)               \
   case cfg::x62_key(WM_, WN_):         \
diff --git a/gaussiank_sgd_amd/ops/csrc/kernels/gemm_units.h b/gaussiank_sgd_amd/ops/csrc/kernels/gemm_units.h
--- a/gaussiank_sgd_amd/ops/csrc/kernels/gemm_units.h
+++ b/gaussiank_sgd_amd/ops/csrc/kernels/gemm_units.h
@@ -24,6 +24,7 @@
   const uint8_t* mask;
   int H, W, OH, OW;
   uint32_t mg_hw, sh_hw, mg_w, sh_w;
+  const void* h2;
 };
 
 inline void magic_u32(uint32_t d, uint32_t* mg, uint32_t* sh) {
diff --git a/gaussiank_sgd_amd/ops/csrc/kernels/gk_kernels.h b/gaussiank_sgd_amd/ops/csrc/kernels/gk_kernels.h
--- a/gaussiank_sgd_amd/ops/csrc/kernels/gk_kernels.h
+++ b/gaussiank_sgd_amd/ops/csrc/kernels/gk_kernels.h
@@ -242,7 +242,7 @@
                          void* fin_state, hipStream_t stream);
 void bn_act_backward_pre_dual(BnShape sh, const void* dz, const void* x, void* dx, const BnBwdStats& bs,
                               BnPartials part, const void* x2, void* dx2, const BnBwdStats& bs2, float* ws2,
-                              hipStream_t stream);
+                              BnPartials part2, hipStream_t stream);
 void bn_act_backward(BnShape sh, const void* dy, const void* dy2, const uint8_t* mask, const void* x, void* dx,
                      void* dres, const BnBwdStats& bs, float* ws, int relu, void* fin_state, hipStream_t stream);
 
@@ -260,6 +260,7 @@
   const void* dy2;
   const uint8_t* mask;
   int H, W, OH, OW;
+  const void* h2;
 };
 struct LazyArgs {
   const void* x;
```

Result: no change. 5011 images/s (-0.9%).
